# apache/arrow-go

Hardware: AMD Instinct MI355X
Metric: GB/s processed per kernel (Sum/Add/Filter/Take) vs HBM roofline (higher is better)
Workload: dtype int64+f64

## Files before the change

arrow_go_amd/csrc/ah_common.h:

```cpp
#pragma once
#include <hip/hip_runtime.h>
#include <initializer_list>
#include <type_traits>
#include <stdarg.h>
#include <stdint.h>
#include <stddef.h>
#include <stdio.h>
#include <stdlib.h>
#include <string.h>
#include "../../include/arrowhip.h"

#define AH_EXPORT extern "C" __attribute__((visibility("default")))

struct ah_filter_cache {
  bool valid;
  const uint8_t *fdata, *fvalid;
  int64_t foff, n, ntiles;
  int null_sel, tile_rows;
  void* buf;
  size_t bytes;
  int64_t* super_off;
  int* tile_local;
  int64_t* total;
};

struct ah_ctx {
  int device;
  hipStream_t stream;
  hipStream_t copy_stream;
  bool owns_stream;
  hipEvent_t ev_copy;
  hipEvent_t ev_compute;
  hipEvent_t t0, t1;
  hipEvent_t* marks;
  int n_marks;
  void* scratch;
  size_t scratch_bytes;
  void* temp;
  size_t temp_bytes;
  void* pack;
  size_t pack_bytes;
  uint64_t* pinned;
  uint64_t* dscalars;
  int num_cu;
  int tune_nt;
  int tune_blocks_per_cu;
  int opt_take_binned, opt_take_window_log2, opt_take_gather_wg, opt_take_gather_load, opt_take_gather_lds;
  int opt_groupby_keys;
  int opt_groupby_partition;
  int opt_encode_partition;
  int opt_encode_part_slots;
  int opt_encode_byte_map;
  int opt_encode_early_look;
  int opt_encode_part_min;
  int opt_hash_direct;
  int opt_hash_sum_partition;
  int opt_sort_msd;
  int opt_scan_segment_log2;
  void* expr_cache;
  int capturing;
  ah_filter_cache fcache;
  int opt_scan_onepass;
  void* scan_recs;
  size_t scan_recs_bytes;
  unsigned scan_epoch;
  int opt_groupby_seed;
  int opt_groupby_reserve;
  int opt_groupby_lean;
  int opt_filter_cache;
  int take_clustered_hint;
  int opt_take_vec;
  bool take_hint_valid, take_hint_live;
  const void* take_hint_idx; int64_t take_hint_nidx; int take_hint_kind, take_hint_near, take_hint_uses, opt_take_hint_cache;
  unsigned long long take_hint_word;
  int opt_arith_xcd_map;
  int opt_groupby_scale_guess;
  int opt_encode_unperm2_group;
  int opt_encode_resolve_wgs;
  int opt_encode_dict_compact;
  int opt_encode_table_batch;
  int opt_encode_unperm_group;
  int opt_take_vec_nt;
  unsigned long long* mailbox;
  unsigned long long mailbox_seq;
  char err[512];
};

static inline unsigned ah_stream_grid(const ah_ctx* c, int64_t work_items, int default_bpc = 8) {
  int bpc = c->tune_blocks_per_cu > 0 ? c->tune_blocks_per_cu : default_bpc;
  int64_t cap = bpc > 0 ? (int64_t)c->num_cu * bpc : ((int64_t)1 << 30);
  int64_t g = work_items < cap ? work_items : cap;
  return (unsigned)(g < 1 ? 1 : g);
}

static inline int ah_fail(ah_ctx* ctx, int code, const char* fmt, ...) __attribute__((format(printf, 3, 4)));
static inline int ah_fail(ah_ctx* ctx, int code, const char* fmt, ...) {
  if (ctx) {
    va_list ap;
    va_start(ap, fmt);
    vsnprintf(ctx->err, sizeof(ctx->err), fmt, ap);
    va_end(ap);
  }
  return code;
}

#define AH_HIP(ctx, call)                                                              \
  do {                                                                                 \
    hipError_t e__ = (call);                                                           \
    if (e__ != hipSuccess)                                                             \
      return ah_fail((ctx), AH_EHIP, "%s failed: %s (%s:%d)", #call, hipGetErrorString(e__), \
                     __FILE__, __LINE__);                                              \
  } while (0)

#define AH_ENTER_KEEP(ctx)                                             \
  do {                                                                 \
    if (!(ctx)) return AH_EINVALID;                                    \
    (ctx)->err[0] = 0;                                                 \
    AH_HIP((ctx), hipSetDevice((ctx)->device));                        \
  } while (0)

#define AH_ENTER(ctx)                                                  \
  do {                                                                 \
    AH_ENTER_KEEP(ctx);                                                \
    (ctx)->fcache.valid = false;                                       \
    (ctx)->take_hint_valid = false;                                    \
  } while (0)

static inline bool ah_take_hint_overlaps(const ah_ctx* c, const void* p, size_t nbytes) {
  if (!c->take_hint_valid || !c->take_hint_idx) return false;
  const uintptr_t a = (uintptr_t)p, b = a + nbytes, lo = (uintptr_t)c->take_hint_idx, hi = lo + (size_t)c->take_hint_nidx * (size_t)(c->take_hint_kind / 2);
  return a < hi && lo < b;
}
static inline bool ah_fcache_overlaps(const ah_ctx* c, const void* p, size_t nbytes) {
  if (!c->fcache.valid) return false;
  const uintptr_t a = (uintptr_t)p, b = a + nbytes;
  const uintptr_t lo = (uintptr_t)(c->fcache.foff >> 3), hi = (uintptr_t)((c->fcache.foff + c->fcache.n + 7) >> 3);
  for (const uint8_t* bm : {c->fcache.fdata, c->fcache.fvalid})
    if (bm && a < (uintptr_t)bm + hi && (uintptr_t)bm + lo < b) return true;
  return false;
}

#define AH_LAUNCH_CHECK(ctx) AH_HIP((ctx), hipGetLastError())

void ah_expr_cache_free(ah_ctx* ctx);
int ah_arith_binary(ah_ctx* ctx, int type, int op, int shape, const void* l, const void* r, void* out, int64_t len);
int ah_partition_by_group(ah_ctx* ctx, const int32_t* ids, const unsigned long long* vals, const uint8_t* vvalid, int64_t voff, int64_t n,
                          int shift, int passes, unsigned* hist, unsigned* offs, unsigned long long* alt_vals, unsigned* alt_ids,
                          unsigned long long* out_vals, unsigned* out_ids);
int ah_sort_rest_msd(ah_ctx* ctx, unsigned long long* keys, unsigned* rows, unsigned long long* alt_keys, unsigned* alt_rows, int64_t n,
                     unsigned long long varying, unsigned long long kmin, unsigned long long kmax, int float_bytes, int descending, void* tmp,
                     unsigned long long* out64, int* used);
size_t ah_sort_msd_temp_bytes(int64_t n);
int ah_sort_pairs_lsd(ah_ctx* ctx, unsigned long long* keys, unsigned* rows, unsigned long long* alt_keys, unsigned* alt_rows, int64_t n,
                      unsigned* hist, unsigned* offs, unsigned long long** sorted_keys);
int ah_take_binned_try(ah_ctx* ctx, int byte_width, const void* values, const uint8_t* vvalid, int64_t voff, int64_t nvalues, int iw,
                       int is_signed, const void* idx, const uint8_t* ivalid, int64_t ioff, int64_t nidx, void* out_values,
                       uint8_t* out_valid, unsigned long long* first_bad, int* used);
int ah_groupby_partitioned_try(ah_ctx* ctx, int is_f64, const uint64_t* keys, const uint8_t* kvalid, int64_t koff, const void* vals,
                               const uint8_t* vvalid, int64_t voff, int64_t n, uint64_t* out_keys, void* out_sums, int64_t* out_counts,
                               int64_t* out_first_rows, int64_t* out_ngroups, int32_t* out_null_group, int* used);
int ah_fused_f64_parts_dev(ah_ctx* ctx, int cmpop, const double* x, const uint8_t* valid, int64_t off, int64_t n, double threshold,
                           double* out_sum_dev, int64_t* out_count_dev, double* out_parts_dev);
size_t ah_sum_partial_bytes(int is_f64);
int ah_sum_chunk_partials(ah_ctx* ctx, int is_f64, const void* buf, size_t len, void* partials, int max_partials, int* n_written);
int ah_sum_finish_partials(ah_ctx* ctx, int is_f64, const void* partials, int n, void* res_dev);
int ah_sum_short_f64(ah_ctx* ctx, const void* buf, size_t len, void* res_dev);
int ah_encode_partitioned_try(ah_ctx* ctx, const uint64_t* keys, const uint8_t* valid, int64_t off, int64_t n, int encode_nulls, int lp, int slots,
                              int32_t* out_ids, uint64_t* out_dict, int64_t* out_first_rows, int64_t* out_ndict, int32_t* out_null_id, int* used);
int ah_encode_u64_groups(ah_ctx* ctx, const uint64_t* keys, const uint8_t* kvalid, int64_t koff, int64_t n, int32_t* ids, uint64_t* out_keys,
                         int64_t* out_first_rows, int64_t* out_ngroups, int32_t* out_null_group);
int ah_encode_u64_first_seen(ah_ctx* ctx, const uint64_t* keys, const uint8_t* valid, int64_t off, int64_t n, int32_t* ids, int64_t* out_first_rows,
                             int64_t* out_ngroups);
int ah_encode_tuple_first_seen(ah_ctx* ctx, int ncols, const ah_group_key* keys, int64_t n, int32_t* ids, int64_t* out_first_rows, int64_t* out_ngroups);
int ah_encode_first_look(ah_ctx* ctx, const uint64_t* keys, const uint8_t* valid, int64_t off, int64_t rows, uint64_t* distinct);
int ah_encode_partitioned2_try(ah_ctx* ctx, const uint64_t* keys, const uint8_t* valid, int64_t off, int64_t n, int encode_nulls, int lp, int slots,
                               int32_t* out_ids, uint64_t* out_dict, int64_t* out_first_rows, int64_t* out_ndict, int32_t* out_null_id, int* used);
int ah_compact_u64_by_bits(ah_ctx* ctx, const uint64_t* values, const uint8_t* bits, int64_t n, uint64_t* out_values, int64_t* out_rows);
int ah_check_stall(ah_ctx* ctx);
int ah_mailbox_read(ah_ctx* ctx, const unsigned long long* dev_words, int nwords, unsigned long long* out_host);
int ah_mailbox_begin(ah_ctx* ctx, unsigned long long** mb_out, unsigned long long* seq_out);
int ah_mailbox_wait(ah_ctx* ctx, unsigned long long seq, int nwords, unsigned long long* out_host);
#if defined(__HIPCC__)
__device__ __forceinline__ void ah_mailbox_post(unsigned long long* mb, unsigned long long seq, const unsigned long long* words, int nwords) {
  for (int i = 0; i < nwords; i++) __hip_atomic_store(&mb[i], words[i], __ATOMIC_RELAXED, __HIP_MEMORY_SCOPE_SYSTEM);
  __hip_atomic_store(&mb[7], seq, __ATOMIC_RELEASE, __HIP_MEMORY_SCOPE_SYSTEM);
}
#endif
int ah_mailbox_read2(ah_ctx* ctx, const unsigned long long* dev_words, int nwords, const unsigned long long* dev_words2, int nwords2,
                     unsigned long long* out_host);
int ah_scratch_reserve(ah_ctx* ctx, size_t nbytes, void** out);
int ah_temp_reserve(ah_ctx* ctx, size_t nbytes, void** out, bool* out_of_memory = nullptr);
int ah_pack_reserve(ah_ctx* ctx, size_t nbytes, void** out);
static inline constexpr size_t ah_pad(size_t b) { return (b + 255) & ~(size_t)255; }
struct TempCarver {
  uint8_t* base = nullptr;
  size_t used = 0;
  uint8_t* take(size_t b) { uint8_t* q = base ? base + used : nullptr; used += ah_pad(b); return q; }
  template <typename T> size_t take(T*& p, size_t count) { p = (T*)take(count * sizeof(T)); return ah_pad(count * sizeof(T)); }
};
constexpr int kDsScalars = 64;
constexpr int kDsSum = 0;
constexpr int kDsFusedSum = 8, kDsFusedCount = 9;
constexpr int kDsMinMax = 12;
constexpr int kDsGbDone = 20;
constexpr int kDsGbFlags = 21, kDsGbTotal = 22, kDsGbNullId = 23;
constexpr int kDsGbRange = 28;
constexpr int kDsEncFlags = 30, kDsEncTotal = 31, kDsEncNullId = 32;
constexpr int kDsEncLook = 33, kDsEncLookDone = 34;
constexpr int kDsEncLargest = 35, kDsEncLargestDone = 36;
constexpr int kDsPopcountPartials = kDsScalars;
constexpr int kPopcountMaxPartials = 4096;
int ah_popcount_async(ah_ctx* ctx, const uint8_t* bits, int64_t off, int64_t nbits, unsigned long long* total_dev);
int ah_popcount_post(ah_ctx* ctx, const uint8_t* bits, int64_t off, int64_t nbits, unsigned long long* total_dev, const unsigned long long* extra_dev,
                     unsigned long long* out_host );
int ah_zero_bytes(ah_ctx* ctx, void* dptr, size_t nbytes);

static inline int ah_type_width(int type) {
  switch (type) {
    case AH_UINT8: case AH_INT8: return 1;
    case AH_UINT16: case AH_INT16: return 2;
    case AH_UINT32: case AH_INT32: case AH_FLOAT32: return 4;
    case AH_UINT64: case AH_INT64: case AH_FLOAT64: return 8;
  }
  return 0;
}

static inline int64_t ah_ceil_div(int64_t a, int64_t b) { return (a + b - 1) / b; }

template <typename T> struct TypeTag { using type = T; };
template <class F>
inline bool with_numeric_type(int type, F&& f) {
  switch (type) {
    case AH_UINT8: f(TypeTag<uint8_t>{}); return true;
    case AH_INT8: f(TypeTag<int8_t>{}); return true;
    case AH_UINT16: f(TypeTag<uint16_t>{}); return true;
    case AH_INT16: f(TypeTag<int16_t>{}); return true;
    case AH_UINT32: f(TypeTag<uint32_t>{}); return true;
    case AH_INT32: f(TypeTag<int32_t>{}); return true;
    case AH_UINT64: f(TypeTag<uint64_t>{}); return true;
    case AH_INT64: f(TypeTag<int64_t>{}); return true;
    case AH_FLOAT32: f(TypeTag<float>{}); return true;
    case AH_FLOAT64: f(TypeTag<double>{}); return true;
  }
  return false;
}
template <class F>
inline bool with_numeric_carrier(int type, F&& f) {
  return with_numeric_type(type, [&](auto t) {
    using T = typename decltype(t)::type;
    if constexpr (__is_floating_point(T)) f(t);
    else f(TypeTag<typename std::make_unsigned<T>::type>{});
  });
}

static inline int ah_flag_clear(ah_ctx* c, unsigned* flag) {
  AH_HIP(c, hipMemsetAsync(flag, 0, sizeof(unsigned), c->stream));
  return AH_OK;
}
static inline int ah_flag_read(ah_ctx* c, const unsigned* flag, unsigned* bits) {
  AH_HIP(c, hipMemcpyAsync(c->pinned, flag, sizeof(unsigned), hipMemcpyDeviceToHost, c->stream));
  AH_HIP(c, hipStreamSynchronize(c->stream));
  *bits = *(volatile unsigned*)c->pinned;
  return AH_OK;
}
int ah_error_of_flag(ah_ctx* ctx, unsigned bits);

#define AH_WAVE 64

template <typename T>
struct alignas(sizeof(T)) ah_vec16 {
  T v[16 / sizeof(T)];
};

template <typename T>
using ah_raw16 __attribute__((aligned(sizeof(T)))) = T __attribute__((ext_vector_type(16 / sizeof(T))));
template <typename T>
__device__ __forceinline__ ah_vec16<T> ah_ld16_nt(const T* p) {
  const ah_raw16<T> raw = __builtin_nontemporal_load(reinterpret_cast<const ah_raw16<T>*>(p));
  ah_vec16<T> r;
#pragma unroll
  for (int j = 0; j < (int)(16 / sizeof(T)); j++) r.v[j] = raw[j];
  return r;
}
template <typename T>
__device__ __forceinline__ void ah_st16_nt(T* p, const ah_vec16<T>& x) {
  ah_raw16<T> raw;
#pragma unroll
  for (int j = 0; j < (int)(16 / sizeof(T)); j++) raw[j] = x.v[j];
  __builtin_nontemporal_store(raw, reinterpret_cast<ah_raw16<T>*>(p));
}

template <typename T>
__device__ __forceinline__ ah_vec16<T> ah_ld16(const T* p) {
  const ah_raw16<T> raw = *reinterpret_cast<const ah_raw16<T>*>(p);
  ah_vec16<T> r;
#pragma unroll
  for (int j = 0; j < (int)(16 / sizeof(T)); j++) r.v[j] = raw[j];
  return r;
}
template <typename T>
__device__ __forceinline__ void ah_st16(T* p, const ah_vec16<T>& x) {
  ah_raw16<T> raw;
#pragma unroll
  for (int j = 0; j < (int)(16 / sizeof(T)); j++) raw[j] = x.v[j];
  *reinterpret_cast<ah_raw16<T>*>(p) = raw;
}

template <typename T>
using ah_aligned16 = T __attribute__((ext_vector_type(16 / sizeof(T))));
template <typename ST>
__device__ __forceinline__ ah_vec16<ST> ah_load16(const ST* base, int64_t i, bool aligned) {
  ah_vec16<ST> v;
  if (aligned) {
    const ah_aligned16<ST> t = __builtin_nontemporal_load((const ah_aligned16<ST>*)base + i);
    __builtin_memcpy(&v, &t, 16);
  } else {
    v = ah_ld16<ST>(base + i * (int64_t)(16 / sizeof(ST)));
  }
  return v;
}
template <typename ST>
__device__ __forceinline__ void ah_store16(ST* base, int64_t i, const ah_vec16<ST>& v, bool aligned) {
  if (aligned) {
    ah_aligned16<ST> t;
    __builtin_memcpy(&t, &v, 16);
    __builtin_nontemporal_store(t, (ah_aligned16<ST>*)base + i);
  } else {
    ah_st16<ST>(base + i * (int64_t)(16 / sizeof(ST)), v);
  }
}

template <typename T>
__device__ __forceinline__ T ah_wave_sum(T v) {
#pragma unroll
  for (int o = 32; o > 0; o >>= 1) v += __shfl_down(v, o, 64);
  return v;
}
template <typename T>
__device__ __forceinline__ T ah_wave_max(T v) {
#pragma unroll
  for (int o = 32; o > 0; o >>= 1) {
    const T t = __shfl_down(v, o, 64);
    v = t > v ? t : v;
  }
  return v;
}
template <typename A, typename B>
__device__ __forceinline__ void ah_wave_max2(A& a, B& b) {
#pragma unroll
  for (int o = 32; o > 0; o >>= 1) {
    const A ta = __shfl_down(a, o, 64);
    const B tb = __shfl_down(b, o, 64);
    a = ta > a ? ta : a;
    b = tb > b ? tb : b;
  }
}

__device__ __forceinline__ int ah_lane() { return (int)(threadIdx.x & 63); }

__device__ __forceinline__ int ah_bit(const uint8_t* __restrict__ bm, int64_t i) {
  return bm == nullptr ? 1 : (bm[i >> 3] >> (i & 7)) & 1;
}

__device__ __forceinline__ uint64_t ah_load_bits64(const uint8_t* __restrict__ bm, int64_t pos, int nvalid);
__device__ __forceinline__ uint64_t ah_wave_bits64(const uint8_t* __restrict__ bm, int64_t pos0, int64_t nrows_left) {
  const int64_t p = ((int64_t)__builtin_amdgcn_readfirstlane((int)(pos0 >> 32)) << 32) | (unsigned)__builtin_amdgcn_readfirstlane((int)pos0);
  const int64_t left = ((int64_t)__builtin_amdgcn_readfirstlane((int)(nrows_left >> 32)) << 32) | (unsigned)__builtin_amdgcn_readfirstlane((int)nrows_left);
  return ah_load_bits64(bm, p, left >= 64 ? 64 : (int)(left < 0 ? 0 : left));
}
__device__ __forceinline__ uint64_t ah_load_bits64(const uint8_t* __restrict__ bm, int64_t pos, int nvalid) {
  uint64_t mask = nvalid >= 64 ? ~0ull : ((1ull << nvalid) - 1);
  if (nvalid <= 0) return 0;
  if (bm == nullptr) return mask;
  uintptr_t addr = (uintptr_t)bm + (uintptr_t)(pos >> 3);
  uintptr_t base = addr & ~(uintptr_t)7;
  int shift = (int)((addr - base) * 8 + (pos & 7));
  const uint64_t* w = (const uint64_t*)base;
  uint64_t lo = w[0] >> shift;
  if (shift != 0 && shift + nvalid > 64) lo |= w[1] << (64 - shift);
  return lo & mask;
}

__device__ __forceinline__ void put_bits(uint8_t* __restrict__ bm, int64_t pos, unsigned long long word, int cnt) {
  const uintptr_t addr = (uintptr_t)bm + (uintptr_t)(pos >> 3);
  const int sub = (int)(pos & 7);
  if (cnt == 64 && sub == 0 && (addr & 7) == 0) {
    *(unsigned long long*)addr = word;
    return;
  }
  const uintptr_t base = addr & ~(uintptr_t)3;
  int shift = (int)((addr - base) * 8) + sub;
  const unsigned long long m = cnt >= 64 ? ~0ull : ((1ull << cnt) - 1);
  word &= m;
  unsigned* w = (unsigned*)base;
  const unsigned long long mlo = m << shift, vlo = word << shift;
  const unsigned long long mhi = shift ? (m >> (64 - shift)) : 0ull, vhi = shift ? (word >> (64 - shift)) : 0ull;
  const unsigned m0 = (unsigned)mlo, m1 = (unsigned)(mlo >> 32), m2 = (unsigned)mhi;
  const unsigned v0 = (unsigned)vlo, v1 = (unsigned)(vlo >> 32), v2 = (unsigned)vhi;
  if (m0) { atomicAnd(&w[0], ~m0); if (v0) atomicOr(&w[0], v0); }
  if (m1) { atomicAnd(&w[1], ~m1); if (v1) atomicOr(&w[1], v1); }
  if (m2) { atomicAnd(&w[2], ~m2); if (v2) atomicOr(&w[2], v2); }
}

__device__ __forceinline__ void put_word(uint8_t* __restrict__ out, int64_t out_off, int aligned, int64_t chunk, unsigned long long word, int cnt) {
  if (aligned && cnt == 64) *(unsigned long long*)(out + (out_off + chunk * 64) / 8) = word;
  else put_bits(out, out_off + chunk * 64, word, cnt);
}

__device__ __forceinline__ void put_chunk_bytes(uint8_t* __restrict__ bm, int64_t chunk, int64_t n, unsigned long long word) {
  const int64_t left = n - chunk * 64;
  const int nbytes = left >= 64 ? 8 : (int)((left + 7) >> 3);
  for (int b = 0; b < nbytes; b++) bm[chunk * 8 + b] = (uint8_t)(word >> (8 * b));
}
```

arrow_go_amd/csrc/ah_ctx.hip:

```cpp
#include <chrono>
#include "ah_common.h"

static const char* kVersion = "arrowhip 0.1 (gfx950)";

AH_EXPORT const char* ah_version(void) { return kVersion; }

AH_EXPORT int ah_device_count(int* n_host) {
  int n = 0;
  hipError_t e = hipGetDeviceCount(&n);
  if (n_host) *n_host = (e == hipSuccess) ? n : 0;
  return e == hipSuccess ? AH_OK : AH_EHIP;
}

static int ctx_init_common(ah_ctx* c) {
  AH_HIP(c, hipStreamCreateWithFlags(&c->copy_stream, hipStreamNonBlocking));
  AH_HIP(c, hipEventCreateWithFlags(&c->ev_copy, hipEventDisableTiming));
  AH_HIP(c, hipEventCreateWithFlags(&c->ev_compute, hipEventDisableTiming));
  AH_HIP(c, hipEventCreate(&c->t0));
  AH_HIP(c, hipEventCreate(&c->t1));
  AH_HIP(c, hipHostMalloc((void**)&c->pinned, 64 * sizeof(uint64_t), hipHostMallocDefault));
  AH_HIP(c, hipMalloc((void**)&c->dscalars, (kDsScalars + kPopcountMaxPartials) * sizeof(uint64_t)));
  AH_HIP(c, hipMemset(c->dscalars, 0, (kDsScalars + kPopcountMaxPartials) * sizeof(uint64_t)));
  AH_HIP(c, hipHostMalloc((void**)&c->mailbox, 256, hipHostMallocCoherent | hipHostMallocMapped));
  memset(c->mailbox, 0, 256);
  hipDeviceProp_t prop;
  AH_HIP(c, hipGetDeviceProperties(&prop, c->device));
  c->num_cu = prop.multiProcessorCount > 0 ? prop.multiProcessorCount : 256;
  const char* e_nt = getenv("ARROWHIP_NT");
  c->tune_nt = e_nt ? atoi(e_nt) : 1;
  const char* e_bpc = getenv("ARROWHIP_BLOCKS_PER_CU");
  c->tune_blocks_per_cu = e_bpc ? atoi(e_bpc) : 0;
  auto env_int = [](const char* name, int dflt) { const char* e = getenv(name); return e ? atoi(e) : dflt; };
  c->opt_take_binned = env_int("ARROWHIP_TAKE_BINNED", 1);
  c->opt_take_window_log2 = env_int("ARROWHIP_TAKE_WINDOW_LOG2", 22);
  c->opt_take_gather_wg = env_int("ARROWHIP_TAKE_GATHER_WG_PER_CU", 8);
  c->opt_groupby_partition = env_int("ARROWHIP_GROUPBY_PARTITION", 1);
  c->opt_groupby_keys = env_int("ARROWHIP_GROUPBY_KEYS", 1280);
  c->opt_hash_direct = env_int("ARROWHIP_HASH_DIRECT", 2);
  c->opt_hash_sum_partition = env_int("ARROWHIP_HASH_PARTITION", 1);
  c->opt_encode_partition = env_int("ARROWHIP_ENCODE_PARTITION", 1);
  c->opt_encode_part_min = env_int("ARROWHIP_ENCODE_PART_MIN", 300000);
  c->opt_encode_early_look = env_int("ARROWHIP_ENCODE_EARLY_LOOK", 1);
  c->opt_encode_byte_map = env_int("ARROWHIP_ENCODE_BYTE_MAP", 1);
  c->opt_encode_part_slots = env_int("ARROWHIP_ENCODE_PART_SLOTS", 8192);
  c->opt_sort_msd = env_int("ARROWHIP_SORT_MSD", 1);
  c->opt_scan_segment_log2 = env_int("ARROWHIP_SCAN_SEGMENT_LOG2", 0);
  c->opt_take_gather_lds = env_int("ARROWHIP_TAKE_GATHER_LDS", 1);
  c->opt_take_vec_nt = env_int("ARROWHIP_TAKE_VEC_NT", 7);
  c->opt_encode_unperm_group = env_int("ARROWHIP_ENCODE_UNPERM_GROUP", 4);
  c->opt_encode_table_batch = env_int("ARROWHIP_ENCODE_TABLE_BATCH", 1);
  c->opt_encode_dict_compact = env_int("ARROWHIP_ENCODE_DICT_COMPACT", 1);
  c->opt_encode_resolve_wgs = env_int("ARROWHIP_ENCODE_RESOLVE_WGS", 1024);
  c->opt_encode_unperm2_group = env_int("ARROWHIP_ENCODE_UNPERM2_GROUP", 4);
  c->opt_groupby_scale_guess = env_int("ARROWHIP_GROUPBY_SCALE_GUESS", 1);
  c->opt_arith_xcd_map = env_int("ARROWHIP_ARITH_XCD_MAP", 0);
  c->opt_take_vec = env_int("ARROWHIP_TAKE_VEC", 1);
  c->opt_take_gather_load = env_int("ARROWHIP_TAKE_GATHER_LOAD", 0);
  return AH_OK;
}

static int ctx_create(int device_id, void* stream, bool borrow, ah_ctx** out) {
  if (!out) return AH_EINVALID;
  *out = nullptr;
  ah_ctx* c = (ah_ctx*)calloc(1, sizeof(ah_ctx));
  if (!c) return AH_EINVALID;
  c->device = device_id;
  hipError_t e = hipSetDevice(device_id);
  if (e != hipSuccess) { free(c); return AH_EHIP; }
  if (borrow) {
    c->stream = (hipStream_t)stream;
    c->owns_stream = false;
  } else {
    e = hipStreamCreateWithFlags(&c->stream, hipStreamNonBlocking);
    if (e != hipSuccess) { free(c); return AH_EHIP; }
    c->owns_stream = true;
  }
  int rc = ctx_init_common(c);
  if (rc != AH_OK) { fprintf(stderr, "arrowhip: ctx init failed: %s\n", c->err); free(c); return rc; }
  c->opt_filter_cache = c->owns_stream ? 1 : 0;
  c->opt_take_hint_cache = c->owns_stream ? 1 : 0;
  c->opt_groupby_lean = 1;
  c->opt_scan_onepass = 1;
  c->opt_groupby_seed = 1;
  c->opt_groupby_reserve = 1;
  *out = c;
  return AH_OK;
}

AH_EXPORT int ah_ctx_create(int device_id, ah_ctx** out) { return ctx_create(device_id, nullptr, false, out); }
AH_EXPORT int ah_ctx_create_on_stream(int device_id, void* hip_stream, ah_ctx** out) {
  return ctx_create(device_id, hip_stream, true, out);
}

AH_EXPORT void ah_ctx_destroy(ah_ctx* c) {
  if (!c) return;
  (void)hipSetDevice(c->device);
  (void)hipStreamSynchronize(c->stream);
  (void)hipStreamSynchronize(c->copy_stream);
  ah_expr_cache_free(c);
  if (c->scratch) (void)hipFree(c->scratch);
  if (c->pinned) (void)hipHostFree(c->pinned);
  if (c->dscalars) (void)hipFree(c->dscalars);
  if (c->mailbox) (void)hipHostFree(c->mailbox);
  if (c->fcache.buf) (void)hipFree(c->fcache.buf);
  if (c->scan_recs) (void)hipFree(c->scan_recs);
  if (c->temp) (void)hipFree(c->temp);
  if (c->pack) (void)hipFree(c->pack);
  (void)hipEventDestroy(c->ev_copy);
  (void)hipEventDestroy(c->ev_compute);
  (void)hipEventDestroy(c->t0);
  (void)hipEventDestroy(c->t1);
  for (int i = 0; i < c->n_marks; i++) if (c->marks[i]) (void)hipEventDestroy(c->marks[i]);
  free(c->marks);
  (void)hipStreamDestroy(c->copy_stream);
  if (c->owns_stream) (void)hipStreamDestroy(c->stream);
  free(c);
}

AH_EXPORT int ah_ctx_set_option(ah_ctx* c, const char* name, int64_t value) {
  AH_ENTER(c);
  if (!name) return ah_fail(c, AH_EINVALID, "set_option: null name");
  if (!strcmp(name, "nt")) c->tune_nt = (int)value;
  else if (!strcmp(name, "blocks_per_cu")) c->tune_blocks_per_cu = (int)value;
  else if (!strcmp(name, "take_binned")) c->opt_take_binned = (int)value;
  else if (!strcmp(name, "take_window_log2")) c->opt_take_window_log2 = (int)value;
  else if (!strcmp(name, "take_gather_wg_per_cu")) c->opt_take_gather_wg = (int)value;
  else if (!strcmp(name, "take_gather_lds")) c->opt_take_gather_lds = (int)value;
  else if (!strcmp(name, "take_vec")) c->opt_take_vec = (int)value;
  else if (!strcmp(name, "take_hint_cache")) { c->opt_take_hint_cache = (int)value; c->take_hint_valid = false; }
  else if (!strcmp(name, "take_vec_nt")) c->opt_take_vec_nt = (int)value;
  else if (!strcmp(name, "encode_unperm_group")) c->opt_encode_unperm_group = (int)value;
  else if (!strcmp(name, "encode_table_batch")) c->opt_encode_table_batch = (int)value;
  else if (!strcmp(name, "encode_dict_compact")) c->opt_encode_dict_compact = (int)value;
  else if (!strcmp(name, "encode_unperm2_group")) c->opt_encode_unperm2_group = (int)value;
  else if (!strcmp(name, "encode_resolve_wgs")) c->opt_encode_resolve_wgs = value < 1 ? 1 : (int)value;
  else if (!strcmp(name, "groupby_scale_guess")) c->opt_groupby_scale_guess = (int)value;
  else if (!strcmp(name, "arith_xcd_map")) c->opt_arith_xcd_map = (int)value;
  else if (!strcmp(name, "take_gather_load")) c->opt_take_gather_load = (int)value;
  else if (!strcmp(name, "groupby_partition")) c->opt_groupby_partition = (int)value;
  else if (!strcmp(name, "groupby_keys")) c->opt_groupby_keys = (int)value;
  else if (!strcmp(name, "hash_direct")) c->opt_hash_direct = (int)value;
  else if (!strcmp(name, "hash_sum_partition")) c->opt_hash_sum_partition = (int)value;
  else if (!strcmp(name, "encode_partition")) c->opt_encode_partition = (int)value;
  else if (!strcmp(name, "encode_part_min")) c->opt_encode_part_min = (int)value;
  else if (!strcmp(name, "encode_early_look")) c->opt_encode_early_look = (int)value;
  else if (!strcmp(name, "encode_byte_map")) c->opt_encode_byte_map = (int)value;
  else if (!strcmp(name, "encode_part_slots")) c->opt_encode_part_slots = (int)value;
  else if (!strcmp(name, "sort_msd")) c->opt_sort_msd = (int)value;
  else if (!strcmp(name, "scan_onepass")) c->opt_scan_onepass = (int)value;
  else if (!strcmp(name, "groupby_lean")) c->opt_groupby_lean = (int)value;
  else if (!strcmp(name, "groupby_seed")) c->opt_groupby_seed = (int)value;
  else if (!strcmp(name, "groupby_reserve")) c->opt_groupby_reserve = (int)value;
  else if (!strcmp(name, "filter_cache")) { c->opt_filter_cache = value != 0; if (!value) c->fcache.valid = false; }
  else if (!strcmp(name, "scan_segment_log2")) c->opt_scan_segment_log2 = (int)value;
  else return ah_fail(c, AH_EINVALID, "set_option: unknown option '%s'", name);
  return AH_OK;
}

AH_EXPORT const char* ah_last_error(ah_ctx* c) { return c ? c->err : "null context"; }

namespace {
__global__ void mailbox_post_kernel(const unsigned long long* __restrict__ src, int nwords, const unsigned long long* __restrict__ src2, int nwords2,
                                    unsigned long long* mailbox, unsigned long long seq) {
  for (int i = 0; i < nwords; i++) __hip_atomic_store(&mailbox[i], src[i], __ATOMIC_RELAXED, __HIP_MEMORY_SCOPE_SYSTEM);
  for (int i = 0; i < nwords2; i++) __hip_atomic_store(&mailbox[nwords + i], src2[i], __ATOMIC_RELAXED, __HIP_MEMORY_SCOPE_SYSTEM);
  __hip_atomic_store(&mailbox[7], seq, __ATOMIC_RELEASE, __HIP_MEMORY_SCOPE_SYSTEM);
}
}
int ah_mailbox_read(ah_ctx* c, const unsigned long long* dev_words, int nwords, unsigned long long* out_host) {
  return ah_mailbox_read2(c, dev_words, nwords, nullptr, 0, out_host);
}
int ah_mailbox_begin(ah_ctx* c, unsigned long long** mb_out, unsigned long long* seq_out) {
  if (c->capturing) { c->capturing = 2; return ah_fail(c, AH_EINVALID, "this call returns a value to the host: it cannot be recorded into a graph"); }
  *mb_out = c->mailbox + 8;
  *seq_out = ++c->mailbox_seq;
  return AH_OK;
}
int ah_mailbox_wait(ah_ctx* c, unsigned long long seq, int nwords, unsigned long long* out_host) {
  if (nwords < 1 || nwords > 7) return ah_fail(c, AH_EINVALID, "mailbox_wait: 1..7 words");
  unsigned long long* mb = c->mailbox + 8;
  bool seen = false;
  const auto t0 = std::chrono::steady_clock::now();
  for (unsigned spin = 0;; spin++) {
    if (__atomic_load_n(&mb[7], __ATOMIC_ACQUIRE) == seq) { seen = true; break; }
    __builtin_ia32_pause();
    if ((spin & 1023u) == 1023u && std::chrono::steady_clock::now() - t0 > std::chrono::milliseconds(5)) break;
  }
  if (!seen) {
    AH_HIP(c, hipStreamSynchronize(c->stream));
    if (__atomic_load_n(&mb[7], __ATOMIC_ACQUIRE) != seq) return ah_fail(c, AH_EHIP, "mailbox_wait: the kernel did not report");
  }
  for (int i = 0; i < nwords; i++) out_host[i] = __atomic_load_n(&mb[i], __ATOMIC_RELAXED);
  return AH_OK;
}
int ah_mailbox_read2(ah_ctx* c, const unsigned long long* dev_words, int nwords, const unsigned long long* dev_words2, int nwords2,
                     unsigned long long* out_host) {
  if (nwords < 1 || nwords2 < 0 || nwords + nwords2 > 7) return ah_fail(c, AH_EINVALID, "mailbox_read: 1..7 words");
  if (c->capturing) { c->capturing = 2; return ah_fail(c, AH_EINVALID, "this call returns a value to the host: it cannot be recorded into a graph"); }
  unsigned long long* mb = c->mailbox + 8;
  const unsigned long long seq = ++c->mailbox_seq;
  mailbox_post_kernel<<<1, 1, 0, c->stream>>>(dev_words, nwords, dev_words2, nwords2, mb, seq);
  AH_LAUNCH_CHECK(c);
  bool seen = false;
  const auto t0 = std::chrono::steady_clock::now();
  for (unsigned spin = 0;; spin++) {
    if (__atomic_load_n(&mb[7], __ATOMIC_ACQUIRE) == seq) { seen = true; break; }
    __builtin_ia32_pause();
    if ((spin & 1023u) == 1023u && std::chrono::steady_clock::now() - t0 > std::chrono::milliseconds(5)) break;
  }
  if (!seen) {
    AH_HIP(c, hipStreamSynchronize(c->stream));
    if (__atomic_load_n(&mb[7], __ATOMIC_ACQUIRE) != seq) return ah_fail(c, AH_EHIP, "mailbox_read: the post kernel did not report");
  }
  for (int i = 0; i < nwords + nwords2; i++) out_host[i] = __atomic_load_n(&mb[i], __ATOMIC_RELAXED);
  return AH_OK;
}

int ah_scratch_reserve(ah_ctx* c, size_t nbytes, void** out) {
  if (nbytes > c->scratch_bytes) {
    AH_HIP(c, hipStreamSynchronize(c->stream));
    if (c->scratch) AH_HIP(c, hipFree(c->scratch));
    c->scratch = nullptr;
    c->scratch_bytes = 0;
    size_t want = (nbytes + ((size_t)1 << 20) - 1) & ~(((size_t)1 << 20) - 1);
    AH_HIP(c, hipMalloc(&c->scratch, want));
    c->scratch_bytes = want;
  }
  *out = c->scratch;
  return AH_OK;
}

int ah_temp_reserve(ah_ctx* c, size_t nbytes, void** out, bool* out_of_memory) {
  if (out_of_memory) *out_of_memory = false;
  if (nbytes > c->temp_bytes) {
    AH_HIP(c, hipStreamSynchronize(c->stream));
    if (c->temp) AH_HIP(c, hipFree(c->temp));
    c->temp = nullptr;
    c->temp_bytes = 0;
    size_t want = (nbytes + ((size_t)1 << 20) - 1) & ~(((size_t)1 << 20) - 1);
    if (hipMalloc(&c->temp, want) != hipSuccess) { (void)hipGetLastError(); if (out_of_memory) *out_of_memory = true; return ah_fail(c, AH_EHIP, "out of device memory (%zu bytes of temporaries)", want); }
    c->temp_bytes = want;
  }
  *out = c->temp;
  return AH_OK;
}

int ah_pack_reserve(ah_ctx* c, size_t nbytes, void** out) {
  if (nbytes > c->pack_bytes) {
    AH_HIP(c, hipStreamSynchronize(c->stream));
    if (c->pack) AH_HIP(c, hipFree(c->pack));
    c->pack = nullptr;
    c->pack_bytes = 0;
    size_t want = (nbytes + ((size_t)1 << 20) - 1) & ~(((size_t)1 << 20) - 1);
    if (hipMalloc(&c->pack, want) != hipSuccess) { (void)hipGetLastError(); return ah_fail(c, AH_EHIP, "out of device memory (%zu bytes of packed keys)", want); }
    c->pack_bytes = want;
  }
  *out = c->pack;
  return AH_OK;
}

AH_EXPORT int ah_buf_alloc(ah_ctx* c, size_t nbytes, void** dptr_host) {
  AH_ENTER_KEEP(c);
  if (!dptr_host) return ah_fail(c, AH_EINVALID, "ah_buf_alloc: null out pointer");
  *dptr_host = nullptr;
  if (nbytes == 0) nbytes = 1;
  nbytes = (nbytes + 63) & ~(size_t)63;
  AH_HIP(c, hipMalloc(dptr_host, nbytes));
  return AH_OK;
}

AH_EXPORT int ah_buf_free(ah_ctx* c, void* dptr) {
  AH_ENTER(c);
  if (dptr) AH_HIP(c, hipFree(dptr));
  return AH_OK;
}

AH_EXPORT int ah_host_alloc_pinned(ah_ctx* c, size_t nbytes, void** hptr_host) {
  AH_ENTER_KEEP(c);
  if (!hptr_host) return ah_fail(c, AH_EINVALID, "ah_host_alloc_pinned: null out pointer");
  if (nbytes == 0) nbytes = 1;
  nbytes = (nbytes + 63) & ~(size_t)63;
  AH_HIP(c, hipHostMalloc(hptr_host, nbytes, hipHostMallocDefault));
  return AH_OK;
}

AH_EXPORT int ah_host_free_pinned(ah_ctx* c, void* hptr) {
  AH_ENTER_KEEP(c);
  if (hptr) AH_HIP(c, hipHostFree(hptr));
  return AH_OK;
}

AH_EXPORT int ah_upload_async(ah_ctx* c, void* dptr, const void* hptr, size_t nbytes) {
  AH_ENTER_KEEP(c);
  if (ah_fcache_overlaps(c, dptr, nbytes)) c->fcache.valid = false;
  if (ah_take_hint_overlaps(c, dptr, nbytes)) c->take_hint_valid = false;
  if (nbytes == 0) return AH_OK;
  AH_HIP(c, hipEventRecord(c->ev_compute, c->stream));
  AH_HIP(c, hipStreamWaitEvent(c->copy_stream, c->ev_compute, 0));
  AH_HIP(c, hipMemcpyAsync(dptr, hptr, nbytes, hipMemcpyHostToDevice, c->copy_stream));
  AH_HIP(c, hipEventRecord(c->ev_copy, c->copy_stream));
  AH_HIP(c, hipStreamWaitEvent(c->stream, c->ev_copy, 0));
  return AH_OK;
}

AH_EXPORT int ah_download_async(ah_ctx* c, void* hptr, const void* dptr, size_t nbytes) {
  AH_ENTER_KEEP(c);
  if (nbytes == 0) return AH_OK;
  AH_HIP(c, hipEventRecord(c->ev_compute, c->stream));
  AH_HIP(c, hipStreamWaitEvent(c->copy_stream, c->ev_compute, 0));
  AH_HIP(c, hipMemcpyAsync(hptr, dptr, nbytes, hipMemcpyDeviceToHost, c->copy_stream));
  AH_HIP(c, hipEventRecord(c->ev_copy, c->copy_stream));
  AH_HIP(c, hipStreamWaitEvent(c->stream, c->ev_copy, 0));
  return AH_OK;
}

AH_EXPORT int ah_memset_async(ah_ctx* c, void* dptr, int byte_value, size_t nbytes) {
  AH_ENTER_KEEP(c);
  if (ah_fcache_overlaps(c, dptr, nbytes)) c->fcache.valid = false;
  if (ah_take_hint_overlaps(c, dptr, nbytes)) c->take_hint_valid = false;
  if (nbytes == 0) return AH_OK;
  AH_HIP(c, hipMemsetAsync(dptr, byte_value, nbytes, c->stream));
  return AH_OK;
}

namespace {
typedef unsigned zero_v4 __attribute__((ext_vector_type(4)));
__global__ __launch_bounds__(256) void zero_bytes_kernel(uint8_t* __restrict__ p, size_t n) {
  const size_t head = ((16 - ((uintptr_t)p & 15)) & 15) < n ? ((16 - ((uintptr_t)p & 15)) & 15) : n;
  const size_t body = (n - head) / 16, tail0 = head + body * 16;
  const size_t i = (size_t)blockIdx.x * 256 + threadIdx.x;
  if (i < head) p[i] = 0;
  if (i < n - tail0) p[tail0 + i] = 0;
  zero_v4* q = (zero_v4*)(p + head);
  const zero_v4 z = {0u, 0u, 0u, 0u};
  for (size_t j = i; j < body; j += (size_t)gridDim.x * 256) q[j] = z;
}
}

int ah_zero_bytes(ah_ctx* c, void* dptr, size_t nbytes) {
  if (nbytes == 0) return AH_OK;
  const size_t want = (nbytes / 16 + 255) / 256 + 1;
  zero_bytes_kernel<<<(unsigned)(want < 4096 ? want : 4096), 256, 0, c->stream>>>((uint8_t*)dptr, nbytes);
  AH_LAUNCH_CHECK(c);
  return AH_OK;
}

namespace {
constexpr int kCopyBlock = 256, kCopyUnroll = 4;
typedef unsigned copy_v4 __attribute__((ext_vector_type(4)));
__global__ __launch_bounds__(kCopyBlock) void copy16_kernel(const copy_v4* __restrict__ src, copy_v4* __restrict__ dst, int64_t nvec) {
  const int64_t i = (int64_t)blockIdx.x * kCopyBlock * kCopyUnroll + threadIdx.x;
  if (i + (int64_t)(kCopyUnroll - 1) * kCopyBlock < nvec) {
    copy_v4 x[kCopyUnroll];
#pragma unroll
    for (int k = 0; k < kCopyUnroll; k++) x[k] = __builtin_nontemporal_load(&src[i + (int64_t)k * kCopyBlock]);
#pragma unroll
    for (int k = 0; k < kCopyUnroll; k++) __builtin_nontemporal_store(x[k], &dst[i + (int64_t)k * kCopyBlock]);
  } else {
#pragma unroll
    for (int k = 0; k < kCopyUnroll; k++) {
      const int64_t j = i + (int64_t)k * kCopyBlock;
      if (j < nvec) dst[j] = src[j];
    }
  }
}
}

AH_EXPORT int ah_copy_async(ah_ctx* c, void* dst, const void* src, size_t nbytes) {
  AH_ENTER_KEEP(c);
  if (ah_fcache_overlaps(c, dst, nbytes)) c->fcache.valid = false;
  if (ah_take_hint_overlaps(c, dst, nbytes)) c->take_hint_valid = false;
  if (nbytes == 0) return AH_OK;
  if (!dst || !src) return ah_fail(c, AH_EINVALID, "copy: null buffer");
  const uintptr_t d = (uintptr_t)dst, s = (uintptr_t)src;
  const bool disjoint = d + nbytes <= s || s + nbytes <= d;
  if (nbytes >= ((size_t)1 << 20) && ((d | s) & 15) == 0 && disjoint) {
    const int64_t nvec = (int64_t)(nbytes / 16);
    copy16_kernel<<<(unsigned)ah_ceil_div(nvec, (int64_t)kCopyBlock * kCopyUnroll), kCopyBlock, 0, c->stream>>>((const copy_v4*)src, (copy_v4*)dst, nvec);
    AH_LAUNCH_CHECK(c);
    const size_t done = (size_t)nvec * 16;
    if (done < nbytes) AH_HIP(c, hipMemcpyAsync((uint8_t*)dst + done, (const uint8_t*)src + done, nbytes - done, hipMemcpyDeviceToDevice, c->stream));
    return AH_OK;
  }
  AH_HIP(c, hipMemcpyAsync(dst, src, nbytes, hipMemcpyDeviceToDevice, c->stream));
  return AH_OK;
}

int ah_check_stall(ah_ctx* c) {
  if (!c->mailbox || !__atomic_load_n(&c->mailbox[16], __ATOMIC_ACQUIRE)) return AH_OK;
  __atomic_store_n(&c->mailbox[16], 0ull, __ATOMIC_RELAXED);
  return ah_fail(c, AH_EHIP, "cumulative_sum: a tile's look-back gave up waiting for a predecessor (results of that call are invalid)");
}

AH_EXPORT int ah_sync(ah_ctx* c) {
  AH_ENTER_KEEP(c);
  AH_HIP(c, hipStreamSynchronize(c->copy_stream));
  AH_HIP(c, hipStreamSynchronize(c->stream));
  return ah_check_stall(c);
}

AH_EXPORT int ah_timer_start(ah_ctx* c) {
  AH_ENTER_KEEP(c);
  AH_HIP(c, hipEventRecord(c->t0, c->stream));
  return AH_OK;
}

AH_EXPORT int ah_timer_stop(ah_ctx* c, float* ms_host) {
  AH_ENTER_KEEP(c);
  AH_HIP(c, hipEventRecord(c->t1, c->stream));
  AH_HIP(c, hipEventSynchronize(c->t1));
  float ms = 0.f;
  AH_HIP(c, hipEventElapsedTime(&ms, c->t0, c->t1));
  if (ms_host) *ms_host = ms;
  return AH_OK;
}

AH_EXPORT int ah_event_record(ah_ctx* c, int slot) {
  AH_ENTER_KEEP(c);
  if (slot < 0 || slot >= (1 << 16)) return ah_fail(c, AH_EINVALID, "event_record: slot out of range");
  if (slot >= c->n_marks) {
    int n = c->n_marks ? c->n_marks : 64;
    while (n <= slot) n *= 2;
    hipEvent_t* m = (hipEvent_t*)realloc(c->marks, (size_t)n * sizeof(hipEvent_t));
    if (!m) return ah_fail(c, AH_EINVALID, "event_record: out of memory");
    for (int i = c->n_marks; i < n; i++) m[i] = nullptr;
    c->marks = m;
    c->n_marks = n;
  }
  if (!c->marks[slot]) AH_HIP(c, hipEventCreate(&c->marks[slot]));
  AH_HIP(c, hipEventRecord(c->marks[slot], c->stream));
  return AH_OK;
}

AH_EXPORT int ah_event_elapsed_ms(ah_ctx* c, int slot_a, int slot_b, float* ms_host) {
  AH_ENTER_KEEP(c);
  if (slot_a < 0 || slot_b < 0 || slot_a >= c->n_marks || slot_b >= c->n_marks || !c->marks[slot_a] || !c->marks[slot_b])
    return ah_fail(c, AH_EINVALID, "event_elapsed_ms: slot never recorded");
  AH_HIP(c, hipEventSynchronize(c->marks[slot_b]));
  float ms = 0.f;
  AH_HIP(c, hipEventElapsedTime(&ms, c->marks[slot_a], c->marks[slot_b]));
  if (ms_host) *ms_host = ms;
  return AH_OK;
}

AH_EXPORT int ah_wait_event(ah_ctx* c, void* hip_event_ptr) {
  AH_ENTER_KEEP(c);
  if (!hip_event_ptr) return AH_OK;
  AH_HIP(c, hipStreamWaitEvent(c->stream, *(hipEvent_t*)hip_event_ptr, 0));
  return AH_OK;
}

AH_EXPORT int ah_device_id(ah_ctx* c) { return c ? c->device : -1; }


struct ah_graph {
  ah_ctx* ctx;
  hipGraph_t graph;
  hipGraphExec_t exec;
  void* scratch;
  void* temp;
};

AH_EXPORT int ah_graph_begin(ah_ctx* c) {
  AH_ENTER(c);
  if (c->capturing) return ah_fail(c, AH_EINVALID, "graph_begin: already capturing");
  AH_HIP(c, hipStreamBeginCapture(c->stream, hipStreamCaptureModeRelaxed));
  c->capturing = 1;
  return AH_OK;
}

AH_EXPORT int ah_graph_end(ah_ctx* c, ah_graph** out) {
  if (!c) return AH_EINVALID;
  c->err[0] = 0;
  if (!out) return ah_fail(c, AH_EINVALID, "graph_end: null out pointer");
  *out = nullptr;
  if (!c->capturing) return ah_fail(c, AH_EINVALID, "graph_end: not capturing");
  const bool poisoned = c->capturing == 2;
  c->capturing = 0;
  hipGraph_t g = nullptr;
  hipError_t e = hipStreamEndCapture(c->stream, &g);
  if (e == hipSuccess && g && poisoned) {
    (void)hipGraphDestroy(g);
    return ah_fail(c, AH_EINVALID, "graph_end: a recorded call needed a value on the host — nothing was run, the capture is dropped");
  }
  if (e != hipSuccess || !g) {
    (void)hipGetLastError();
    return ah_fail(c, AH_EHIP, "graph_end: the capture was invalidated (%s) — a captured call waited for the device or allocated", hipGetErrorString(e));
  }
  hipGraphExec_t x = nullptr;
  e = hipGraphInstantiate(&x, g, nullptr, nullptr, 0);
  if (e != hipSuccess) { (void)hipGraphDestroy(g); return ah_fail(c, AH_EHIP, "graph_end: hipGraphInstantiate failed: %s", hipGetErrorString(e)); }
  ah_graph* r = (ah_graph*)calloc(1, sizeof(ah_graph));
  if (!r) { (void)hipGraphExecDestroy(x); (void)hipGraphDestroy(g); return ah_fail(c, AH_EINVALID, "graph_end: out of memory"); }
  r->ctx = c; r->graph = g; r->exec = x;
  r->scratch = c->scratch; r->temp = c->temp;
  *out = r;
  return AH_OK;
}

AH_EXPORT int ah_graph_launch(ah_ctx* c, ah_graph* g) {
  AH_ENTER(c);
  if (!g || g->ctx != c) return ah_fail(c, AH_EINVALID, "graph_launch: not a graph of this context");
  if (c->capturing) return ah_fail(c, AH_EINVALID, "graph_launch: the context is capturing");
  if (g->scratch != c->scratch || g->temp != c->temp)
    return ah_fail(c, AH_EINVALID, "graph_launch: a call since the recording grew one of the context's work areas (the recorded launches point into the old block) — record the sequence again");
  AH_HIP(c, hipGraphLaunch(g->exec, c->stream));
  return AH_OK;
}

AH_EXPORT int ah_graph_destroy(ah_graph* g) {
  if (!g) return AH_OK;
  (void)hipSetDevice(g->ctx->device);
  (void)hipStreamSynchronize(g->ctx->stream);
  (void)hipGraphExecDestroy(g->exec);
  (void)hipGraphDestroy(g->graph);
  free(g);
  return AH_OK;
}
```

arrow_go_amd/csrc/ah_msd.h:

```cpp
#pragma once
#include "ah_common.h"
#include "ah_bins.h"

namespace {

constexpr int kMsTile = 4096;
constexpr int kMsRows = kMsTile / kThreads;
constexpr int kMaxNb2 = 2048;

struct TileRange { int64_t lo, hi, id; int parent; };
__device__ __forceinline__ int ms_parent_of(int j, int nparents) { const int per = nparents >> 3; return ((j % per) << 3) | (j / per); }
__device__ __forceinline__ unsigned ms_tiles_of(const unsigned* __restrict__ pstart, const unsigned* __restrict__ pend, int j, int nparents) {
  const int p = ms_parent_of(j, nparents);
  return ((pend ? pend[p] : pstart[p + 1]) - pstart[p] + kMsTile - 1) / kMsTile;
}
__device__ __forceinline__ void ms_parent_tiles(const unsigned* __restrict__ pstart, const unsigned* __restrict__ pend, int nparents, unsigned* s_cnt,
                                                unsigned* s_start, unsigned* s_wsum) {
  const int t = threadIdx.x;
  s_cnt[t] = t < nparents ? ms_tiles_of(pstart, pend, t, nparents) : 0u;
  __syncthreads();
  block_excl_scan(s_cnt, s_start, s_wsum, nparents);
}
__device__ __forceinline__ long long ms_block_tile(unsigned b, unsigned nblocks, int nparents, const unsigned* s_cnt, const unsigned* s_start) {
  const int per = nparents >> 3;
  const unsigned x = b & 7, q = b >> 3, nblk = nblocks >> 3;
  auto class_lo = [&](unsigned c) { return s_start[c * per]; };
  auto class_n = [&](unsigned c) { return (c == 7 ? s_start[nparents - 1] + s_cnt[nparents - 1] : s_start[(c + 1) * per]) - s_start[c * per]; };
  long long g = -1;
  if (q < class_n(x)) {
    g = class_lo(x) + q;
  } else {
    unsigned spare = q - class_n(x);
    for (unsigned c = 0; c < x; c++) spare += nblk > class_n(c) ? nblk - class_n(c) : 0u;
    for (unsigned c = 0; c < 8 && g < 0; c++) {
      const unsigned surplus = class_n(c) > nblk ? class_n(c) - nblk : 0u;
      if (spare < surplus) g = class_lo(c) + nblk + spare; else spare -= surplus;
    }
  }
  return g;
}
__device__ __forceinline__ TileRange ms_tile_of_parent(const unsigned* __restrict__ pstart, const unsigned* __restrict__ pend, int nparents, int j, long long g,
                                                       const unsigned* s_start) {
  TileRange r;
  const int p = ms_parent_of(j, nparents);
  const int64_t b0 = pstart[p], b1 = pend ? pend[p] : pstart[p + 1];
  r.lo = b0 + (int64_t)(g - s_start[j]) * kMsTile;
  r.hi = r.lo + kMsTile < b1 ? r.lo + kMsTile : b1;
  r.id = g;
  r.parent = p;
  return r;
}
__device__ __forceinline__ TileRange ms_tile(const unsigned* __restrict__ pstart, int nparents, int64_t n, unsigned* s_cnt, unsigned* s_start,
                                             unsigned* s_wsum, int* s_pick, const unsigned* __restrict__ pend = nullptr) {
  TileRange r{0, 0, 0, -1};
  if (!pstart) {
    const int64_t tile = xcd_contiguous_tile((n + kMsTile - 1) / kMsTile);
    if (tile >= 0) { r.lo = tile * kMsTile; r.hi = r.lo + kMsTile < n ? r.lo + kMsTile : n; r.id = tile; r.parent = 0; }
    return r;
  }
  const int t = threadIdx.x;
  if (t == 0) *s_pick = -1;
  ms_parent_tiles(pstart, pend, nparents, s_cnt, s_start, s_wsum);
  const long long g = ms_block_tile(blockIdx.x, gridDim.x, nparents, s_cnt, s_start);
  if (g >= 0 && t < nparents && s_cnt[t] && s_start[t] <= g && g < s_start[t] + s_cnt[t]) *s_pick = t;
  __syncthreads();
  const int j = *s_pick;
  return j < 0 ? r : ms_tile_of_parent(pstart, pend, nparents, j, g, s_start);
}

__global__ __launch_bounds__(kThreads) void ms_tile_table_kernel(const unsigned* __restrict__ pstart, const unsigned* __restrict__ pend, int nparents,
                                                                  unsigned nblocks, TileRange* __restrict__ table) {
  __shared__ unsigned s_cnt[kThreads], s_start[kThreads], s_wsum[kThreads / 64];
  ms_parent_tiles(pstart, pend, nparents, s_cnt, s_start, s_wsum);
  const unsigned b = blockIdx.x * (unsigned)kThreads + threadIdx.x;
  if (b >= nblocks) return;
  const long long g = ms_block_tile(b, nblocks, nparents, s_cnt, s_start);
  TileRange r{0, 0, 0, -1};
  if (g >= 0) {
    int lo = 0, hi = nparents - 1;
    while (lo < hi) { const int mid = (lo + hi + 1) >> 1; if ((long long)s_start[mid] <= g) lo = mid; else hi = mid - 1; }
    int j = lo;
    while (j > 0 && !s_cnt[j]) j--;
    if (s_cnt[j] && (long long)s_start[j] <= g && g < (long long)s_start[j] + s_cnt[j]) r = ms_tile_of_parent(pstart, pend, nparents, j, g, s_start);
  }
  table[b] = r;
}

template <typename DIGIT>
__global__ __launch_bounds__(kThreads) void tile_hist_kernel(DIGIT dg, int64_t n, const unsigned* __restrict__ pstart, int nparents, int nb,
                                                              unsigned* __restrict__ cnt, const TileRange* __restrict__ tile_table = nullptr) {
  __shared__ unsigned s_h[DIGIT::kMaxDigits];
  __shared__ unsigned s_cnt[kThreads], s_start[kThreads], s_wsum[kThreads / 64];
  __shared__ int s_pick;
  const TileRange r = tile_table ? tile_table[blockIdx.x] : ms_tile(pstart, nparents, n, s_cnt, s_start, s_wsum, &s_pick);
  if (r.parent < 0) return;
  for (int b = threadIdx.x; b < nb; b += kThreads) s_h[b] = 0;
  __syncthreads();
  unsigned d[kMsRows];
#pragma unroll
  for (int u = 0; u < kMsRows; u++) { const int64_t i = r.lo + u * kThreads + threadIdx.x; d[u] = i < r.hi ? dg.digit(i, r.parent) : 0u; }
#pragma unroll
  for (int u = 0; u < kMsRows; u++) { const int64_t i = r.lo + u * kThreads + threadIdx.x; if (i < r.hi) atomicAdd(&s_h[d[u]], 1u); }
  __syncthreads();
  for (int b = threadIdx.x; b < nb; b += kThreads) cnt[r.id * nb + b] = s_h[b];
}

__global__ __launch_bounds__(kThreads) void ms_offs2_kernel(const unsigned* __restrict__ cnt, const unsigned* __restrict__ pstart, int nparents, int nb,
                                                             unsigned* __restrict__ toffs, unsigned* __restrict__ bstart, int64_t n,
                                                             unsigned* __restrict__ largest = nullptr, unsigned* __restrict__ done = nullptr,
                                                             unsigned long long* mb = nullptr, unsigned long long seq = 0) {
  __shared__ unsigned s_cnt[kThreads], s_start[kThreads], s_wsum[kThreads / 64];
  __shared__ unsigned s_carry;
  const int t = threadIdx.x, p = blockIdx.x;
  ms_parent_tiles(pstart, nullptr, nparents, s_cnt, s_start, s_wsum);
  const int j = (p & 7) * (nparents >> 3) + (p >> 3);
  const int64_t vt0 = s_start[j], vt1 = vt0 + s_cnt[j];
  __syncthreads();
  const unsigned base = pstart[p];
  auto post_largest = [&](unsigned mine) {
    if (!largest) return;
    if (t == 0) s_carry = 0;
    __syncthreads();
    if (mine) atomicMax(&s_carry, mine);
    __syncthreads();
    if (t == 0) {
      atomicMax(largest, s_carry);
      __threadfence();
      if (atomicAdd(done, 1u) == gridDim.x - 1u) {
        __threadfence();
        const unsigned long long w = __hip_atomic_exchange(largest, 0u, __ATOMIC_RELAXED, __HIP_MEMORY_SCOPE_AGENT);
        __hip_atomic_store(done, 0u, __ATOMIC_RELAXED, __HIP_MEMORY_SCOPE_AGENT);
        ah_mailbox_post(mb, seq, &w, 1);
      }
    }
  };
  if (nb <= kThreads / 2) {
    const int d = t & (nb - 1), g = t / nb, G = kThreads / nb;
    const int64_t per = (vt1 - vt0 + G - 1) / G, a0 = vt0 + g * per, a1 = a0 + per < vt1 ? a0 + per : vt1;
    unsigned part = 0;
    for (int64_t vt = a0; vt < a1; vt++) part += cnt[vt * nb + d];
    s_cnt[t] = part;
    __syncthreads();
    unsigned before = 0, tot = 0;
    for (int gg = 0; gg < G; gg++) { const unsigned c = s_cnt[gg * nb + d]; before += gg < g ? c : 0u; tot += c; }
    __syncthreads();
    s_cnt[t] = t < nb ? tot : 0u;
    __syncthreads();
    block_excl_scan(s_cnt, s_start, s_wsum, nb);
    post_largest(t < nb ? tot : 0u);
    unsigned run = base + s_start[d] + before;
    if (g == 0) bstart[(int64_t)p * nb + d] = run;
    for (int64_t vt = a0; vt < a1; vt++) { toffs[vt * nb + d] = run; run += cnt[vt * nb + d]; }
    if (p == nparents - 1 && t == 0) bstart[(int64_t)nparents * nb] = (unsigned)n;
    return;
  }
  unsigned tot[2] = {0, 0};
  for (int64_t vt = vt0; vt < vt1; vt++)
    for (int h = 0; h < 2; h++) { const int d = t + h * kThreads; if (d < nb) tot[h] += cnt[vt * nb + d]; }
  unsigned excl[2];
  unsigned carry = 0;
  for (int h = 0; h < 2; h++) {
    if (h * kThreads >= nb) break;
    s_cnt[t] = t + h * kThreads < nb ? tot[h] : 0u;
    __syncthreads();
    block_excl_scan(s_cnt, s_start, s_wsum, kThreads);
    excl[h] = carry + s_start[t];
    if (t == kThreads - 1) s_carry = s_start[t] + s_cnt[t];
    __syncthreads();
    carry += s_carry;
    __syncthreads();
  }
  post_largest(tot[0] > tot[1] ? tot[0] : tot[1]);
  for (int h = 0; h < 2; h++) {
    const int d = t + h * kThreads;
    if (d >= nb) break;
    unsigned run = base + excl[h];
    bstart[(int64_t)p * nb + d] = run;
    for (int64_t vt = vt0; vt < vt1; vt++) { toffs[vt * nb + d] = run; run += cnt[vt * nb + d]; }
  }
  if (p == nparents - 1 && t == 0) bstart[(int64_t)nparents * nb] = (unsigned)n;
}

template <int CTRL>
__device__ __forceinline__ unsigned ms_dpp(unsigned v) { return (unsigned)__builtin_amdgcn_update_dpp((int)v, (int)v, CTRL, 0xF, 0xF, false); }
__device__ __forceinline__ unsigned ms_xor_lane(unsigned v, int j, int lane) {
  switch (j) {
    case 1: return ms_dpp<0xB1>(v);
    case 2: return ms_dpp<0x4E>(v);
    case 4: { const unsigned a = ms_dpp<0x124>(v), b = ms_dpp<0x12C>(v); return (lane & 4) ? a : b; }
    case 8: return ms_dpp<0x128>(v);
    case 16: { auto r = __builtin_amdgcn_permlane16_swap(v, v, false, false); return (lane & 16) ? r[0] : r[1]; }
    default: { auto r = __builtin_amdgcn_permlane32_swap(v, v, false, false); return (lane & 32) ? r[0] : r[1]; }
  }
}
template <typename E>
__device__ __forceinline__ E ms_pick(const E& mine, const E& other, bool keep_min) {
  const bool other_less = E::less(other, mine);
  return (other_less == keep_min) ? other : mine;
}

template <typename E, int SLOTS>
__device__ __forceinline__ void ms_bitonic(E (&x)[SLOTS], int lane) {
#pragma unroll
  for (int k = 2; k <= 64 * SLOTS; k <<= 1) {
#pragma unroll
    for (int j = k >> 1; j > 0; j >>= 1) {
      if (j >= 64) {
#pragma unroll
        for (int sl = 0; sl < SLOTS; sl++) {
          const int ps = sl ^ (j >> 6);
          if (ps > sl) {
            const bool asc = (sl & (k >> 6)) == 0;
            const bool swap = E::less(x[ps], x[sl]) == asc;
            const E a = x[sl], bb = x[ps];
            x[sl] = swap ? bb : a;
            x[ps] = swap ? a : bb;
          }
        }
      } else {
        const bool low = (lane & j) == 0;
#pragma unroll
        for (int sl = 0; sl < SLOTS; sl++) {
          const bool asc = k < 64 ? (lane & k) == 0 : (sl & (k >> 6)) == 0;
          x[sl] = ms_pick(x[sl], E::xchg(x[sl], j, lane), low == asc);
        }
      }
    }
  }
}
}
```

arrow_go_amd/csrc/ah_sort.hip:

```cpp
#include <algorithm>
#include <type_traits>
#include <vector>
#include "ah_sort_radix.h"

namespace {

enum { kCatRest = 0, kCatNaN = 1, kCatNull = 2 };

template <typename T>
__device__ __forceinline__ unsigned long long make_key(T v, bool descending) {
  using U = typename std::make_unsigned<typename std::conditional<std::is_floating_point<T>::value,
                                                                    typename std::conditional<sizeof(T) == 4, int, long long>::type, T>::type>::type;
  constexpr U sign = (U)1 << (sizeof(T) * 8 - 1);
  U k;
  if constexpr (std::is_floating_point<T>::value) {
    if (v == (T)0) v = (T)0;
    U b = __builtin_bit_cast(U, v);
    k = (b & sign) ? (U)~b : (U)(b | sign);
  } else if constexpr (std::is_signed<T>::value) {
    k = (U)v ^ sign;
  } else {
    k = (U)v;
  }
  if (descending) k = (U)~k;
  return (unsigned long long)k;
}

template <typename T>
struct Column {
  const T* values;
  const uint8_t* valid;
  int64_t off;
  int descending, nulls_at_start;
  const unsigned* rows_in;
  __device__ __forceinline__ void load(int64_t i, unsigned long long* key, unsigned* row, unsigned* digit) const {
    const unsigned r = rows_in ? rows_in[i] : (unsigned)i;
    const T v = values[r];
    int cat = kCatRest;
    if (!ah_bit(valid, off + r)) cat = kCatNull;
    else if (std::is_floating_point<T>::value && v != v) cat = kCatNaN;
    *key = cat == kCatRest ? make_key<T>(v, descending) : 0ull;
    *row = r;
    *digit = nulls_at_start ? (unsigned)(2 - cat) : (unsigned)cat;
  }
};
struct IdVal {
  const int32_t* ids;
  const unsigned long long* vals;
  const uint8_t* vvalid;
  int64_t voff;
  int shift;
  __device__ __forceinline__ void load(int64_t i, unsigned long long* key, unsigned* row, unsigned* digit) const {
    const unsigned g = (unsigned)ids[i];
    const bool ok = ah_bit(vvalid, voff + i);
    *key = ok ? vals[i] : 0ull;
    *row = ok ? g : (g | 0x80000000u);
    *digit = (g >> shift) & 255u;
  }
};

struct ValId {
  const unsigned long long* vals;
  const unsigned* ids;
  int shift;
  __device__ __forceinline__ void load(int64_t i, unsigned long long* key, unsigned* row, unsigned* digit) const {
    *key = vals[i];
    *row = ids[i];
    *digit = ((*row & 0x7fffffffu) >> shift) & 255u;
  }
};

template <typename T>
__global__ __launch_bounds__(kBlock) void pairs_kernel(const T* __restrict__ values, int64_t n, int descending, unsigned long long* __restrict__ keys,
                                                        unsigned* __restrict__ rows, unsigned long long* __restrict__ res) {
  KeyStats st;
  st.init();
  constexpr int U = 4;
  const int64_t stride = (int64_t)gridDim.x * kBlock * U;
  for (int64_t base = (int64_t)blockIdx.x * kBlock * U + threadIdx.x; base < n; base += stride) {
    T v[U];
#pragma unroll
    for (int u = 0; u < U; u++) { const int64_t i = base + (int64_t)u * kBlock; v[u] = i < n ? __builtin_nontemporal_load(&values[i]) : (T)0; }
#pragma unroll
    for (int u = 0; u < U; u++) {
      const int64_t i = base + (int64_t)u * kBlock;
      if (i >= n) continue;
      if (std::is_floating_point<T>::value && v[u] != v[u]) { st.nans++; continue; }
      const unsigned long long k = make_key<T>(v[u], descending);
      __builtin_nontemporal_store(k, &keys[i]);
      __builtin_nontemporal_store((unsigned)i, &rows[i]);
      st.add(k);
    }
  }
  st = ah_block_reduce<kBlock>(st);
  if (threadIdx.x == 0) st.store<5>(res + (size_t)blockIdx.x * 5);
}

__global__ __launch_bounds__(kBlock) void emit_kernel(const unsigned* __restrict__ rows, int64_t n, uint64_t* __restrict__ out) {
  const int64_t stride = (int64_t)gridDim.x * kBlock;
  for (int64_t i = (int64_t)blockIdx.x * kBlock + threadIdx.x; i < n; i += stride) out[i] = rows[i];
}


template <typename T>
int sort_by_column(ah_ctx* c, SortBuffers& b, const void* values, const uint8_t* valid, int64_t off, int64_t n, int descending,
                   int nulls_at_start, const unsigned* rows_in) {
  const int64_t ntiles = ah_ceil_div(n, (int64_t)kTile * tiles_per_block(n));
  int rc;
  Column<T> col{(const T*)values, valid, off, descending, nulls_at_start, rows_in};
  int64_t rest_lo = 0, rest_n = 0;
  unsigned long long k_and = ~0ull, k_or = 0, kmin = ~0ull, kmax = 0;
  bool have_stats = false;
  if (valid == nullptr && rows_in == nullptr && n >= ((int64_t)1 << 20)) {
    const unsigned pgrid = std::min(ah_stream_grid(c, ah_ceil_div(n, (int64_t)kBlock * 4), 8), (unsigned)kAndOrGrid);
    pairs_kernel<T><<<pgrid, kBlock, 0, c->stream>>>((const T*)values, n, descending, b.ka, b.ra, b.andor);
    AH_LAUNCH_CHECK(c);
    std::vector<unsigned long long> parts((size_t)pgrid * 5);
    AH_HIP(c, hipMemcpyAsync(parts.data(), b.andor, parts.size() * 8, hipMemcpyDeviceToHost, c->stream));
    AH_HIP(c, hipStreamSynchronize(c->stream));
    unsigned long long nans = 0;
    for (unsigned g = 0; g < pgrid; g++) {
      k_and &= parts[g * 5]; k_or |= parts[g * 5 + 1];
      kmin = parts[g * 5 + 2] < kmin ? parts[g * 5 + 2] : kmin;
      kmax = parts[g * 5 + 3] > kmax ? parts[g * 5 + 3] : kmax;
      nans += parts[g * 5 + 4];
    }
    if (nans == 0) { have_stats = true; rest_lo = 0; rest_n = n; }
  }
  if (!have_stats) {
    if ((rc = radix_pass(c, col, n, b.hist, b.offs, b.ka, b.ra)) != AH_OK) return rc;
    unsigned ends[3];
    for (int d = 0; d < 3; d++)
      AH_HIP(c, hipMemcpyAsync(&c->pinned[d], b.offs + ((int64_t)d + 1) * ntiles - 1, 4, hipMemcpyDeviceToHost, c->stream));
    AH_HIP(c, hipStreamSynchronize(c->stream));
    for (int d = 0; d < 3; d++) ends[d] = *(volatile unsigned*)&c->pinned[d];
    rest_lo = nulls_at_start ? ends[1] : 0;
    rest_n = nulls_at_start ? (int64_t)ends[2] - ends[1] : ends[0];
  }
  unsigned long long *kcur = b.ka + rest_lo, *kalt = b.kb + rest_lo;
  unsigned *rcur = b.ra + rest_lo, *ralt = b.rb + rest_lo;
  if (rest_n > 1) {
    if (!have_stats) {
      const unsigned agrid = std::min(ah_stream_grid(c, ah_ceil_div(rest_n, kBlock), 4), (unsigned)kAndOrGrid);
      and_or_kernel<<<agrid, kBlock, 0, c->stream>>>(kcur, rest_n, b.andor);
      AH_LAUNCH_CHECK(c);
      std::vector<unsigned long long> parts((size_t)agrid * 4);
      AH_HIP(c, hipMemcpyAsync(parts.data(), b.andor, parts.size() * 8, hipMemcpyDeviceToHost, c->stream));
      AH_HIP(c, hipStreamSynchronize(c->stream));
      for (unsigned g = 0; g < agrid; g++) {
        k_and &= parts[g * 4]; k_or |= parts[g * 4 + 1];
        kmin = parts[g * 4 + 2] < kmin ? parts[g * 4 + 2] : kmin;
        kmax = parts[g * 4 + 3] > kmax ? parts[g * 4 + 3] : kmax;
      }
    }
    const unsigned long long varying = k_and ^ k_or;
    int nvar = 0;
    for (int by = 0; by < (int)sizeof(T); by++) nvar += ((varying >> (8 * by)) & 0xFFull) != 0;
    bool done = false;
    if (rows_in == nullptr && nvar >= 4 && c->opt_sort_msd) {
      int used = -1;
      if ((rc = ah_sort_rest_msd(c, kcur, rcur, kalt, ralt, rest_n, varying, kmin, kmax, std::is_floating_point<T>::value ? (int)sizeof(T) : 0, descending, b.msd_tmp,
                                 (unsigned long long*)(rest_n == n ? b.final_out : nullptr), &used)) != AH_OK) return rc;
      if (used > 0) {
        done = true;
        b.emitted = rest_n == n && b.final_out != nullptr;
      } else if (used == 0 && b.msd_tmp && ah_sort_msd_temp_bytes(rest_n) != 0) {
        if ((rc = radix_pass(c, col, n, b.hist, b.offs, b.ka, b.ra)) != AH_OK) return rc;
      }
    }
    for (int by = 0; !done && by < (int)sizeof(T); by++) {
      if (((varying >> (8 * by)) & 0xFFull) == 0) continue;
      Pairs src{kcur, rcur, 8 * by};
      if ((rc = radix_pass(c, src, rest_n, b.hist, b.offs, kalt, ralt)) != AH_OK) return rc;
      unsigned long long* tk = kcur; kcur = kalt; kalt = tk;
      unsigned* tr = rcur; rcur = ralt; ralt = tr;
    }
    if (!b.emitted && rcur != b.ra + rest_lo) AH_HIP(c, hipMemcpyAsync(b.ra + rest_lo, rcur, (size_t)rest_n * 4, hipMemcpyDeviceToDevice, c->stream));
  }
  return AH_OK;
}

int sort_dispatch(ah_ctx* c, SortBuffers& b, const SortCol& k, int64_t n, const unsigned* rows_in) {
  switch (k.type) {
#define AH_SORT(ID, T) case ID: return sort_by_column<T>(c, b, k.values, k.valid, k.off, n, k.descending, k.nulls_at_start, rows_in);
    AH_SORT(AH_UINT8, uint8_t) AH_SORT(AH_INT8, int8_t) AH_SORT(AH_UINT16, uint16_t) AH_SORT(AH_INT16, int16_t)
    AH_SORT(AH_UINT32, uint32_t) AH_SORT(AH_INT32, int32_t) AH_SORT(AH_UINT64, uint64_t) AH_SORT(AH_INT64, int64_t)
    AH_SORT(AH_FLOAT32, float) AH_SORT(AH_FLOAT64, double)
#undef AH_SORT
  }
  if (ah_sort_is_binary(k.type)) return ah_sort_by_binary(c, b, k, n, rows_in);
  return ah_fail(c, AH_ENOTIMPL, "sorting not supported for type %d", k.type);
}

int sort_keys(ah_ctx* c, int nkeys, const SortCol* keys, int64_t n, uint64_t* out) {
  SortBuffers b;
  const int64_t ntiles = ah_ceil_div(n, kTile);
  int rc;
  bool any_binary = false;
  for (int k = 0; k < nkeys; k++) any_binary |= ah_sort_is_binary(keys[k].type);
  const size_t hist_bytes = (size_t)kRadix * ntiles * 4;
  const size_t msd_bytes = c->opt_sort_msd ? ah_sort_msd_temp_bytes(n) : 0;
  const size_t bin_bytes = any_binary ? kBinArrays * Carver::pad((size_t)n * 4) : 0;
  const size_t total = 2 * Carver::pad((size_t)n * 8) + (nkeys > 1 ? 3 : 2) * Carver::pad((size_t)n * 4) + 2 * Carver::pad(hist_bytes) + Carver::pad(4096 * 8 * 8) + Carver::pad(msd_bytes) + bin_bytes;
  void* arena;
  if ((rc = ah_temp_reserve(c, total, &arena)) != AH_OK) return rc;
  Carver tmp{(uint8_t*)arena};
  tmp.take((size_t)n * 8, &b.ka);
  tmp.take((size_t)n * 8, &b.kb);
  tmp.take((size_t)n * 4, &b.ra);
  tmp.take((size_t)n * 4, &b.rb);
  b.rc = nullptr;
  if (nkeys > 1) tmp.take((size_t)n * 4, &b.rc);
  tmp.take(hist_bytes, &b.hist);
  tmp.take(hist_bytes, &b.offs);
  tmp.take((size_t)kAndOrGrid * 8 * 8, &b.andor);
  if (msd_bytes) { uint8_t* m; tmp.take(msd_bytes, &m); b.msd_tmp = m; }
  if (any_binary)
    for (int i = 0; i < kBinArrays; i++) tmp.take((size_t)n * 4, &b.bin[i]);
  const unsigned* rows_in = nullptr;
  if (nkeys == 1) b.final_out = out;
  for (int k = nkeys - 1; k >= 0; k--) {
    if ((rc = sort_dispatch(c, b, keys[k], n, rows_in)) != AH_OK) return rc;
    if (k > 0) {
      AH_HIP(c, hipMemcpyAsync(b.rc, b.ra, (size_t)n * 4, hipMemcpyDeviceToDevice, c->stream));
      rows_in = b.rc;
    }
  }
  if (!b.emitted) {
    emit_kernel<<<ah_stream_grid(c, ah_ceil_div(n, kBlock), 8), kBlock, 0, c->stream>>>(b.ra, n, out);
    AH_LAUNCH_CHECK(c);
  }
  return AH_OK;
}

}

int ah_partition_by_group(ah_ctx* c, const int32_t* ids, const unsigned long long* vals, const uint8_t* vvalid, int64_t voff, int64_t n, int shift,
                          int passes, unsigned* hist, unsigned* offs, unsigned long long* alt_vals, unsigned* alt_ids,
                          unsigned long long* out_vals, unsigned* out_ids) {
  IdVal src{ids, vals, vvalid, voff, shift};
  if (passes == 1) return radix_pass(c, src, n, hist, offs, out_vals, out_ids);
  int rc = radix_pass(c, src, n, hist, offs, alt_vals, alt_ids);
  if (rc != AH_OK) return rc;
  ValId src2{alt_vals, alt_ids, shift + 8};
  return radix_pass(c, src2, n, hist, offs, out_vals, out_ids);
}

int ah_sort_pairs_lsd(ah_ctx* c, unsigned long long* keys, unsigned* rows, unsigned long long* alt_keys, unsigned* alt_rows, int64_t n,
                      unsigned* hist, unsigned* offs, unsigned long long** sorted_keys) {
  for (int by = 0; by < 8; by++) {
    Pairs src{keys, rows, 8 * by};
    int rc = radix_pass(c, src, n, hist, offs, alt_keys, alt_rows);
    if (rc != AH_OK) return rc;
    unsigned long long* tk = keys; keys = alt_keys; alt_keys = tk;
    unsigned* tr = rows; rows = alt_rows; alt_rows = tr;
  }
  *sorted_keys = keys;
  return AH_OK;
}

static int check_column(ah_ctx* c, int type, const void* values) {
  const int w = ah_type_width(type);
  if (!w) return ah_fail(c, AH_ENOTIMPL, "sorting not supported for type %d", type);
  if (!values) return ah_fail(c, AH_EINVALID, "sort_indices: null buffer");
  if ((uintptr_t)values & (uintptr_t)(w - 1)) return ah_fail(c, AH_EINVALID, "sort_indices: buffer not element-aligned");
  return AH_OK;
}

static int check_key(ah_ctx* c, const ah_sort_key& k, SortCol* col) {
  *col = SortCol{k.type, nullptr, nullptr, nullptr, 0, k.valid, k.off, k.descending, k.nulls_at_start};
  switch (k.type) {
    case AH_BINARY: case AH_LARGE_BINARY: {
      const int ow = k.type == AH_BINARY ? 4 : 8;
      if (!k.offsets) return ah_fail(c, AH_EINVALID, "sort_indices: null buffer");
      if ((uintptr_t)k.offsets & (uintptr_t)(ow - 1)) return ah_fail(c, AH_EINVALID, "sort_indices: buffer not element-aligned");
      col->offsets = k.offsets;
      col->data = (const uint8_t*)k.values;
      return AH_OK;
    }
    case AH_FIXED_SIZE_BINARY: case AH_DECIMAL128: case AH_DECIMAL256: {
      const int w = k.type == AH_DECIMAL128 ? 16 : k.type == AH_DECIMAL256 ? 32 : k.byte_width;
      if (k.byte_width != w || w < 1) return ah_fail(c, AH_EINVALID, "sort_indices: byte width %d does not fit type %d", k.byte_width, k.type);
      if (!k.values) return ah_fail(c, AH_EINVALID, "sort_indices: null buffer");
      col->data = (const uint8_t*)k.values;
      col->width = w;
      return AH_OK;
    }
  }
  const int rc = check_column(c, k.type, k.values);
  if (rc != AH_OK) return rc;
  col->values = (const uint8_t*)k.values + k.off * ah_type_width(k.type);
  return AH_OK;
}

AH_EXPORT int ah_sort_indices(ah_ctx* c, int type, const void* values, const uint8_t* valid, int64_t off, int64_t n, int descending,
                              int nulls_at_start, uint64_t* out_indices) {
  return ah_sort_indices_multi(c, 1, &type, &values, &valid, &off, n, &descending, &nulls_at_start, out_indices);
}

AH_EXPORT int ah_sort_indices_multi(ah_ctx* c, int nkeys, const int* types, const void* const* values, const uint8_t* const* valids,
                                    const int64_t* offs, int64_t n, const int* descending, const int* nulls_at_start, uint64_t* out_indices) {
  AH_ENTER(c);
  if (nkeys < 1) return ah_fail(c, AH_EINVALID, "must provide at least one sort key");
  if (n < 0) return ah_fail(c, AH_EINVALID, "sort_indices: negative length");
  for (int k = 0; k < nkeys; k++)
    if (offs[k] < 0) return ah_fail(c, AH_EINVALID, "sort_indices: negative offset");
  if (n == 0) return AH_OK;
  if (!out_indices) return ah_fail(c, AH_EINVALID, "sort_indices: null buffer");
  if (n >= ((int64_t)1 << 32)) return ah_fail(c, AH_ENOTIMPL, "sort_indices: more than 2^32 - 1 rows in one batch");
  std::vector<SortCol> cols((size_t)nkeys);
  for (int k = 0; k < nkeys; k++) {
    int rc = check_column(c, types[k], values[k]);
    if (rc != AH_OK) return rc;
    cols[k] = SortCol{types[k], values[k], nullptr, nullptr, 0, valids[k], offs[k], descending[k], nulls_at_start[k]};
  }
  return sort_keys(c, nkeys, cols.data(), n, out_indices);
}

AH_EXPORT int ah_sort_indices_keys(ah_ctx* c, int nkeys, const ah_sort_key* keys, int64_t n, uint64_t* out_indices) {
  AH_ENTER(c);
  if (nkeys < 1) return ah_fail(c, AH_EINVALID, "must provide at least one sort key");
  if (!keys) return ah_fail(c, AH_EINVALID, "sort_indices: null buffer");
  if (n < 0) return ah_fail(c, AH_EINVALID, "sort_indices: negative length");
  for (int k = 0; k < nkeys; k++)
    if (keys[k].off < 0) return ah_fail(c, AH_EINVALID, "sort_indices: negative offset");
  if (n == 0) return AH_OK;
  if (!out_indices) return ah_fail(c, AH_EINVALID, "sort_indices: null buffer");
  if (n >= ((int64_t)1 << 32)) return ah_fail(c, AH_ENOTIMPL, "sort_indices: more than 2^32 - 1 rows in one batch");
  std::vector<SortCol> cols((size_t)nkeys);
  for (int k = 0; k < nkeys; k++) {
    const int rc = check_key(c, keys[k], &cols[k]);
    if (rc != AH_OK) return rc;
  }
  return sort_keys(c, nkeys, cols.data(), n, out_indices);
}
```

arrow_go_amd/csrc/ah_sort_msd.hip:

```cpp
#include "ah_common.h"
#include "ah_bins.h"
#include "ah_msd.h"

namespace {

constexpr int kLocalMax = 512;
constexpr int kBigMax = 8192, kBigList = 1024;

struct MsMap {
  unsigned long long mask;
  int lshift;
  int fkind, descending;
};
__device__ __forceinline__ double ms_value(unsigned long long u, const MsMap& m) {
  if (m.fkind == 8) {
    const unsigned long long k = m.descending ? ~u : u;
    return __builtin_bit_cast(double, (k >> 63) ? (k & 0x7fffffffffffffffull) : ~k);
  }
  const unsigned k = m.descending ? ~(unsigned)(u >> 32) : (unsigned)(u >> 32);
  return (double)__builtin_bit_cast(float, (k >> 31) ? (k & 0x7fffffffu) : ~k);
}
__device__ __forceinline__ double ms_frac(unsigned long long u, unsigned long long pa, unsigned long long pb, const MsMap& m) {
  if (pb <= pa) return 0.0;
  if (m.fkind && m.lshift == (m.fkind == 8 ? 0 : 32) && ((pa ^ pb) >> 63)) {
    const double xa = ms_value(pa, m), xb = ms_value(pb, m);
    if (xb != xa && xa - xa == 0.0 && xb - xb == 0.0) return (ms_value(u, m) - xa) / (xb - xa);
  }
  return (double)(u - pa) / (double)(pb - pa);
}
constexpr int kSplit = 4096;
constexpr int64_t kSample = (int64_t)1 << 18;

__global__ __launch_bounds__(256) void ms_sample_kernel(const unsigned long long* __restrict__ keys, int64_t n, int64_t stride, int64_t count, MsMap m,
                                                         unsigned long long* __restrict__ sample, unsigned* __restrict__ sample_rows) {
  const int64_t j = (int64_t)blockIdx.x * 256 + threadIdx.x;
  if (j >= count) return;
  const int64_t i = j * stride;
  sample[j] = i < n ? (keys[i] & m.mask) << m.lshift : ~0ull;
  sample_rows[j] = (unsigned)j;
}
struct MsPoints {
  const unsigned long long* sorted;
  int64_t count;
  unsigned long long umin, umax;
  __device__ __forceinline__ unsigned long long at(int64_t i) const { return i <= 0 ? umin : (i > count ? umax : sorted[i - 1]); }
  __device__ __forceinline__ int64_t first(int k) const { return k == 0 ? 0 : 64 * (int64_t)k + 1; }
  __device__ __forceinline__ int64_t last(int k) const { return k == kSplit - 1 ? count + 1 : 64 * (int64_t)(k + 1) + 1; }
};
constexpr int kFlagWords = kSplit / 32;
__global__ __launch_bounds__(256) void ms_split_kernel(MsPoints p, unsigned long long* __restrict__ split, unsigned* __restrict__ flags) {
  const int k = blockIdx.x * 256 + threadIdx.x;
  if (k > kSplit) return;
  split[k] = k == kSplit ? p.umax : p.at(p.first(k));
  if (k == kSplit) return;
  const int64_t i0 = p.first(k), i1 = p.last(k);
  const unsigned long long a = p.at(i0), b = p.at(i1);
  bool flag = k == 0 || k == kSplit - 1;
  if (!flag && b > a) {
    const double w = (double)(b - a), g = (double)(i1 - i0);
    for (int64_t i = i0 + 1; i < i1; i++) {
      const double dev = (double)(p.at(i) - a) / w - (double)(i - i0) / g;
      flag = flag || dev > 0.25 || dev < -0.25;
    }
  }
  if (flag) atomicOr(&flags[k >> 5], 1u << (k & 31));
}

__global__ __launch_bounds__(256) void ms_dupes_kernel(const unsigned long long* __restrict__ sorted, int64_t count, int64_t run, unsigned* __restrict__ found) {
  const int64_t i = (int64_t)blockIdx.x * 256 + threadIdx.x;
  if (i + run < count && sorted[i] == sorted[i + run]) *found = 1u;
}

__global__ __launch_bounds__(256) void ms_guide_kernel(const unsigned long long* __restrict__ split, unsigned short* __restrict__ guide) {
  const int c = blockIdx.x * 256 + threadIdx.x;
  if (c > 4096) return;
  if (c == 4096) { guide[c] = (unsigned short)(kSplit - 1); return; }
  const unsigned long long v = (unsigned long long)c << 52;
  int lo = 0;
  for (int step = kSplit >> 1; step > 0; step >>= 1) lo += split[lo + step] <= v ? step : 0;
  guide[c] = (unsigned short)lo;
}

__global__ __launch_bounds__(kThreads) void ms_bucket_kernel(const unsigned long long* __restrict__ keys, int64_t n, MsMap m, MsPoints p,
                                                         const unsigned long long* __restrict__ split, const unsigned* __restrict__ flags,
                                                         const unsigned short* __restrict__ guide, unsigned per, unsigned* __restrict__ bucket) {
  __shared__ unsigned long long s_s[kSplit + 1];
  __shared__ unsigned s_f[kFlagWords];
  __shared__ unsigned short s_g[4097];
  for (int i = threadIdx.x; i <= kSplit; i += kThreads) { s_s[i] = split[i]; s_g[i] = guide[i]; }
  for (int i = threadIdx.x; i < kFlagWords; i += kThreads) s_f[i] = flags[i];
  __syncthreads();
  constexpr int U = 4;
  const int64_t stride = (int64_t)gridDim.x * kThreads * U;
  for (int64_t base = (int64_t)blockIdx.x * kThreads * U + threadIdx.x; base < n; base += stride) {
    unsigned long long u[U];
    unsigned lo[U], hi[U];
#pragma unroll
    for (int q = 0; q < U; q++) {
      const int64_t i = base + q * kThreads;
      u[q] = i < n ? (__builtin_nontemporal_load(&keys[i]) & m.mask) << m.lshift : s_s[0];
    }
#pragma unroll
    for (int q = 0; q < U; q++) { lo[q] = s_g[u[q] >> 52]; hi[q] = s_g[(u[q] >> 52) + 1]; }
    bool more = true;
    while (more) {
      more = false;
#pragma unroll
      for (int q = 0; q < U; q++) {
        if (lo[q] < hi[q]) {
          const unsigned mid = (lo[q] + hi[q] + 1) >> 1;
          if (s_s[mid] <= u[q]) lo[q] = mid; else hi[q] = mid - 1;
          more = more || lo[q] < hi[q];
        }
      }
    }
#pragma unroll
    for (int q = 0; q < U; q++) {
      const int64_t i = base + q * kThreads;
      if (i >= n) continue;
      double f;
      if ((s_f[lo[q] >> 5] >> (lo[q] & 31)) & 1u) {
        int64_t a = p.first((int)lo[q]), b = p.last((int)lo[q]);
        const double g = (double)(b - a);
        const int64_t a0 = a;
        unsigned long long pa = p.at(a), pb = p.at(b);
        while (b - a > 1) {
          const int64_t mid = (a + b) >> 1;
          const unsigned long long pm = p.at(mid);
          if (b - a <= 16) {
            const double d = ms_frac(pm, pa, pb, m) - (double)(mid - a) / (double)(b - a);
            if (d < 0.3 && d > -0.3) break;
          }
          if (pm <= u[q]) { a = mid; pa = pm; } else { b = mid; pb = pm; }
        }
        f = ((double)(a - a0) + ms_frac(u[q], pa, pb, m) * (double)(b - a)) / g;
      } else {
        const unsigned long long x = s_s[lo[q]], y = s_s[lo[q] + 1];
        f = y > x ? (double)(u[q] - x) * __builtin_amdgcn_rcp((double)(y - x)) : 0.0;
      }
      f = f >= 0.0 ? f : 0.0;
      unsigned in = (unsigned)(f * (double)per);
      in = in < per ? in : per - 1;
      __builtin_nontemporal_store(lo[q] * per + in, &bucket[i]);
    }
  }
}

struct MsDigit {
  static constexpr int kMaxDigits = kMaxNb2;
  const unsigned* bucket; int shift; unsigned mask;
  __device__ __forceinline__ unsigned digit(int64_t i, int) const { return (__builtin_nontemporal_load(&bucket[i]) >> shift) & mask; }
};

template <bool WITH_BUCKET>
__global__ __launch_bounds__(kThreads) void ms_scatter_kernel(const unsigned long long* __restrict__ keys, const unsigned* __restrict__ rows,
                                                               const unsigned* __restrict__ bucket, int64_t n, const unsigned* __restrict__ pstart,
                                                               int nparents, int shift, unsigned mask, int nb, const unsigned* __restrict__ toffs,
                                                               unsigned long long* __restrict__ out_keys, unsigned* __restrict__ out_rows,
                                                               unsigned* __restrict__ out_bucket) {
  __shared__ unsigned s_cnt[kMaxNb2], s_start[kMaxNb2], s_goff[kMaxNb2], s_wsum[kThreads / 64];
  __shared__ unsigned s_a[kThreads], s_b[kThreads];
  __shared__ unsigned long long s_stage[kMsTile];
  __shared__ uint16_t s_bin[kMsTile];
  __shared__ int s_pick;
  __shared__ unsigned s_carry;
  const TileRange r = ms_tile(pstart, nparents, n, s_a, s_b, s_wsum, &s_pick);
  if (r.parent < 0) return;
  const int t = threadIdx.x;
  for (int b = t; b < nb; b += kThreads) s_cnt[b] = 0;
  unsigned long long k[kMsRows];
  unsigned rw[kMsRows], bk[kMsRows], dg[kMsRows], rank[kMsRows];
  bool live[kMsRows];
#pragma unroll
  for (int u = 0; u < kMsRows; u++) {
    const int64_t i = r.lo + u * kThreads + t;
    live[u] = i < r.hi;
    k[u] = live[u] ? __builtin_nontemporal_load(&keys[i]) : 0ull;
    rw[u] = live[u] ? __builtin_nontemporal_load(&rows[i]) : 0u;
    bk[u] = live[u] ? __builtin_nontemporal_load(&bucket[i]) : 0u;
  }
  __syncthreads();
#pragma unroll
  for (int u = 0; u < kMsRows; u++) {
    dg[u] = (bk[u] >> shift) & mask;
    rank[u] = live[u] ? atomicAdd(&s_cnt[dg[u]], 1u) : 0u;
  }
  __syncthreads();
  digit_excl_scan(s_cnt, nb, s_a, s_b, s_wsum, &s_carry, [&](int d, unsigned st) {
    s_start[d] = st;
    s_goff[d] = toffs[r.id * nb + d] - st;
  });
  const int tile_n = (int)(r.hi - r.lo);
#pragma unroll
  for (int u = 0; u < kMsRows; u++)
    if (live[u]) { const unsigned q = s_start[dg[u]] + rank[u]; s_stage[q] = k[u]; s_bin[q] = (uint16_t)dg[u]; }
  __syncthreads();
  int64_t dst[kMsRows];
#pragma unroll
  for (int u = 0; u < kMsRows; u++) {
    const int q = u * kThreads + t;
    dst[u] = q < tile_n ? (int64_t)s_goff[s_bin[q]] + q : -1;
    if (dst[u] >= 0) out_keys[dst[u]] = s_stage[q];
  }
  __syncthreads();
  unsigned* s_stage32 = reinterpret_cast<unsigned*>(s_stage);
#pragma unroll
  for (int u = 0; u < kMsRows; u++)
    if (live[u]) { const unsigned q = s_start[dg[u]] + rank[u]; s_stage32[q] = rw[u]; if (WITH_BUCKET) s_stage32[kMsTile + q] = bk[u]; }
  __syncthreads();
#pragma unroll
  for (int u = 0; u < kMsRows; u++)
    if (dst[u] >= 0) {
      out_rows[dst[u]] = s_stage32[u * kThreads + t];
      if (WITH_BUCKET) out_bucket[dst[u]] = s_stage32[kMsTile + u * kThreads + t];
    }
}

struct KR {
  unsigned long long k;
  unsigned r;
  static __device__ __forceinline__ bool less(const KR& a, const KR& b) { return a.k < b.k || (a.k == b.k && a.r < b.r); }
  static __device__ __forceinline__ KR xchg(const KR& a, int j, int lane) {
    KR o;
    o.k = ((unsigned long long)ms_xor_lane((unsigned)(a.k >> 32), j, lane) << 32) | ms_xor_lane((unsigned)a.k, j, lane);
    o.r = ms_xor_lane(a.r, j, lane);
    return o;
  }
};
__device__ __forceinline__ bool kr_less(const KR& a, const KR& b) { return KR::less(a, b); }
struct C64 {
  unsigned long long c;
  static __device__ __forceinline__ bool less(const C64& a, const C64& b) { return a.c < b.c; }
  static __device__ __forceinline__ C64 xchg(const C64& a, int j, int lane) {
    C64 o;
    o.c = ((unsigned long long)ms_xor_lane((unsigned)(a.c >> 32), j, lane) << 32) | ms_xor_lane((unsigned)a.c, j, lane);
    return o;
  }
};
constexpr int kMsRowBits = 27;
template <int SLOTS>
__device__ __forceinline__ void ms_sort_bucket(const unsigned long long* __restrict__ keys, const unsigned* rows, unsigned s, int m,
                                               int lane, unsigned* out_rows, unsigned long long* __restrict__ out64) {
  KR x[SLOTS];
#pragma unroll
  for (int sl = 0; sl < SLOTS; sl++) {
    const int i = sl * 64 + lane;
    x[sl].k = i < m ? keys[s + i] : ~0ull;
    x[sl].r = i < m ? rows[s + i] : ~0u;
  }
  auto emit = [&](int i, unsigned row) { if (i < m) { if (out64) out64[s + i] = row; else out_rows[s + i] = row; } };
  if (SLOTS <= 2) {
    const unsigned long long k0 = ((unsigned long long)__builtin_amdgcn_readfirstlane((unsigned)(x[0].k >> 32)) << 32) |
                                  __builtin_amdgcn_readfirstlane((unsigned)x[0].k);
    bool fits1 = true, fits2 = true;
#pragma unroll
    for (int sl = 0; sl < SLOTS; sl++) {
      const bool in = sl * 64 + lane < m;
      fits1 = fits1 && (!in || x[sl].k - k0 + (1ull << 36) < (1ull << 37));
      fits2 = fits2 && (!in || x[sl].k - k0 + (1ull << 56) < (1ull << 57));
    }
    if (__all(fits1)) {
      C64 y[SLOTS];
#pragma unroll
      for (int sl = 0; sl < SLOTS; sl++)
        y[sl].c = sl * 64 + lane < m ? ((x[sl].k - k0 + (1ull << 36)) << kMsRowBits) | x[sl].r : ~0ull;
      ms_bitonic<C64, SLOTS>(y, lane);
#pragma unroll
      for (int sl = 0; sl < SLOTS; sl++) emit(sl * 64 + lane, (unsigned)y[sl].c & ((1u << kMsRowBits) - 1u));
      return;
    }
    if (__all(fits2)) {
      C64 y[SLOTS];
#pragma unroll
      for (int sl = 0; sl < SLOTS; sl++)
        y[sl].c = sl * 64 + lane < m ? ((x[sl].k - k0 + (1ull << 56)) << 7) | (unsigned)(sl * 64 + lane) : ~0ull;
      ms_bitonic<C64, SLOTS>(y, lane);
      bool tie = false;
#pragma unroll
      for (int sl = 0; sl < SLOTS; sl++) {
        unsigned long long nxt = __shfl_down(y[sl].c, 1, 64);
        if (sl + 1 < SLOTS) {
          const unsigned long long head = ((unsigned long long)__builtin_amdgcn_readfirstlane((unsigned)(y[sl + 1 < SLOTS ? sl + 1 : sl].c >> 32)) << 32) |
                                          __builtin_amdgcn_readfirstlane((unsigned)y[sl + 1 < SLOTS ? sl + 1 : sl].c);
          nxt = lane == 63 ? head : nxt;
        } else if (lane == 63) {
          nxt = ~0ull;
        }
        tie = tie || (sl * 64 + lane + 1 < m && (y[sl].c >> 7) == (nxt >> 7));
      }
      if (!__any(tie)) {
#pragma unroll
        for (int sl = 0; sl < SLOTS; sl++) {
          const unsigned at = (unsigned)y[sl].c & 127u;
          unsigned row = __shfl(x[0].r, (int)(at & 63u), 64);
          if (SLOTS > 1) { const unsigned row1 = __shfl(x[SLOTS > 1 ? 1 : 0].r, (int)(at & 63u), 64); row = (at >> 6) ? row1 : row; }
          emit(sl * 64 + lane, row);
        }
        return;
      }
    }
  }
  ms_bitonic<KR, SLOTS>(x, lane);
#pragma unroll
  for (int sl = 0; sl < SLOTS; sl++) emit(sl * 64 + lane, x[sl].r);
}

__global__ __launch_bounds__(256) void ms_local_kernel(const unsigned long long* __restrict__ keys, const unsigned* rows,
                                                        const unsigned* __restrict__ bstart, int64_t nbuckets, unsigned* out_rows,
                                                        unsigned long long* __restrict__ out64, unsigned* __restrict__ oversize,
                                                        unsigned* __restrict__ big_list) {
  const int lane = threadIdx.x & 63;
  const int64_t b = (int64_t)blockIdx.x * 4 + (threadIdx.x >> 6);
  if (b >= nbuckets) return;
  const unsigned s = bstart[b], e = bstart[b + 1];
  const int m = (int)(e - s);
  if (m <= 0) return;
  if (m > kLocalMax) {
    if (lane == 0) {
      if (m > kBigMax) atomicMax(&oversize[0], (unsigned)m);
      else { const unsigned at = atomicAdd(&oversize[1], 1u); if (at < (unsigned)kBigList) big_list[at] = (unsigned)b; }
    }
    return;
  }
  if (m == 1) { if (lane == 0) { if (out64) out64[s] = rows[s]; else out_rows[s] = rows[s]; } return; }
  if (m <= 64) ms_sort_bucket<1>(keys, rows, s, m, lane, out_rows, out64);
  else if (m <= 128) ms_sort_bucket<2>(keys, rows, s, m, lane, out_rows, out64);
  else if (m <= 256) ms_sort_bucket<4>(keys, rows, s, m, lane, out_rows, out64);
  else ms_sort_bucket<8>(keys, rows, s, m, lane, out_rows, out64);
}

__global__ __launch_bounds__(kThreads) void ms_big_kernel(const unsigned long long* __restrict__ keys, const unsigned* rows,
                                                           const unsigned* __restrict__ bstart, const unsigned* __restrict__ oversize,
                                                           const unsigned* __restrict__ big_list, unsigned* out_rows,
                                                           unsigned long long* __restrict__ out64) {
  __shared__ unsigned long long s_k[kBigMax];
  __shared__ unsigned s_r[kBigMax];
  if (blockIdx.x >= oversize[1] || blockIdx.x >= (unsigned)kBigList) return;
  const unsigned b = big_list[blockIdx.x], s = bstart[b];
  const int m = (int)(bstart[b + 1] - s);
  int p2 = 1024;
  while (p2 < m) p2 <<= 1;
  for (int i = threadIdx.x; i < p2; i += kThreads) { s_k[i] = i < m ? keys[s + i] : ~0ull; s_r[i] = i < m ? rows[s + i] : ~0u; }
  __syncthreads();
  for (int k = 2; k <= p2; k <<= 1) {
    for (int j = k >> 1; j > 0; j >>= 1) {
      for (int i = threadIdx.x; i < p2; i += kThreads) {
        const int q = i ^ j;
        if (q > i) {
          const KR x{s_k[i], s_r[i]}, y{s_k[q], s_r[q]};
          const bool asc = (i & k) == 0;
          if (kr_less(y, x) == asc) { s_k[i] = y.k; s_r[i] = y.r; s_k[q] = x.k; s_r[q] = x.r; }
        }
      }
      __syncthreads();
    }
  }
  for (int i = threadIdx.x; i < m; i += kThreads) { if (out64) out64[s + i] = s_r[i]; else out_rows[s + i] = s_r[i]; }
}

}

static void ms_plan(int64_t n, int* lb_out, int* lb2_out) {
  int lb = 0;
  while (((int64_t)64 << lb) < n) lb++;
  if (lb > 21) lb = 21;
  *lb_out = lb;
  *lb2_out = lb >= 20 ? lb - 10 : lb - lb / 2;
}

size_t ah_sort_msd_temp_bytes(int64_t n) {
  if (n < ((int64_t)1 << 22) || n > ((int64_t)1 << 27)) return 0;
  int lb, lb2;
  ms_plan(n, &lb, &lb2);
  const int nb2 = 1 << lb2, nb1 = 1 << (lb - lb2);
  const int64_t ntiles = ah_ceil_div(n, kMsTile), ngrp = ah_ceil_div(ntiles, kGroupTiles), nvt = ((ntiles + nb1 + 7) / 8) * 8;
  return ah_pad((size_t)n * 4) * 2 + ah_pad((size_t)kSample * 8) * 2 + ah_pad((size_t)kSample * 4) * 2 + ah_pad((size_t)(kSplit + 1) * 8) + ah_pad(kFlagWords * 4) + ah_pad(4097 * 2) +
         ah_pad((size_t)ntiles * nb1 * 4) * 2 + ah_pad((size_t)ngrp * nb1 * 4) + ah_pad((size_t)(nb1 + 1) * 4) + ah_pad((size_t)nvt * nb2 * 4) * 2 +
         ah_pad(((size_t)1 << lb) * 4 + 4) + ah_pad((size_t)kBigList * 4) + 256;
}

int ah_sort_rest_msd(ah_ctx* c, unsigned long long* keys, unsigned* rows, unsigned long long* alt_keys, unsigned* alt_rows, int64_t n,
                     unsigned long long varying, unsigned long long kmin, unsigned long long kmax, int float_bytes, int descending, void* tmp,
                     unsigned long long* out64, int* used) {
  *used = -1;
  if (!tmp || varying == 0 || ah_sort_msd_temp_bytes(n) == 0) return AH_OK;
  unsigned* out_rows = rows;
  int lb, lb2;
  ms_plan(n, &lb, &lb2);
  const int nb2 = 1 << lb2, nb1 = 1 << (lb - lb2);
  const unsigned nbuckets = 1u << lb;
  const int hb = 63 - __builtin_clzll(varying);
  MsMap map{hb == 63 ? ~0ull : ((1ull << (hb + 1)) - 1), 63 - hb, float_bytes, descending};
  const int64_t ntiles = ah_ceil_div(n, kMsTile), ngrp = ah_ceil_div(ntiles, kGroupTiles), nvt = ((ntiles + nb1 + 7) / 8) * 8;
  const unsigned grid1 = (unsigned)(((ntiles + 7) / 8) * 8);
  const int64_t sample_n = n < kSample ? n : kSample;
  TempCarver tc;
  tc.base = (uint8_t*)tmp;
  int rc;
  unsigned* bucket = (unsigned*)tc.take((size_t)n * 4);
  unsigned* bucket2 = (unsigned*)tc.take((size_t)n * 4);
  unsigned long long* sample = (unsigned long long*)tc.take((size_t)kSample * 8);
  unsigned long long* sample_alt = (unsigned long long*)tc.take((size_t)kSample * 8);
  unsigned* sample_rows = (unsigned*)tc.take((size_t)kSample * 4);
  unsigned* sample_rows_alt = (unsigned*)tc.take((size_t)kSample * 4);
  unsigned long long* split = (unsigned long long*)tc.take((size_t)(kSplit + 1) * 8);
  unsigned* flags = (unsigned*)tc.take(kFlagWords * 4);
  unsigned short* guide = (unsigned short*)tc.take(4097 * 2);
  unsigned* cnt1 = (unsigned*)tc.take((size_t)ntiles * nb1 * 4);
  unsigned* toffs1 = (unsigned*)tc.take((size_t)ntiles * nb1 * 4);
  unsigned* gsum = (unsigned*)tc.take((size_t)ngrp * nb1 * 4);
  unsigned* pstart = (unsigned*)tc.take((size_t)(nb1 + 1) * 4);
  unsigned* cnt2 = (unsigned*)tc.take((size_t)nvt * nb2 * 4);
  unsigned* toffs2 = (unsigned*)tc.take((size_t)nvt * nb2 * 4);
  unsigned* bstart = (unsigned*)tc.take(((size_t)nbuckets + 1) * 4);
  unsigned* big_list = (unsigned*)tc.take((size_t)kBigList * 4);
  unsigned* oversize = (unsigned*)&c->dscalars[26];
  AH_HIP(c, hipMemsetAsync(oversize, 0, 8, c->stream));
  ms_sample_kernel<<<(unsigned)ah_ceil_div(sample_n, 256), 256, 0, c->stream>>>(keys, n, n / sample_n, sample_n, map, sample, sample_rows);
  AH_LAUNCH_CHECK(c);
  unsigned long long* sorted = nullptr;
  if ((rc = ah_sort_pairs_lsd(c, sample, sample_rows, sample_alt, sample_rows_alt, sample_n, (unsigned*)cnt2, (unsigned*)toffs2, &sorted)) != AH_OK) return rc;
  {
    const int64_t run = (int64_t)(kBigMax / 2) * sample_n / n;
    ms_dupes_kernel<<<(unsigned)ah_ceil_div(sample_n, 256), 256, 0, c->stream>>>(sorted, sample_n, run < 1 ? 1 : run, oversize);
    AH_LAUNCH_CHECK(c);
    AH_HIP(c, hipMemcpyAsync(&c->pinned[12], oversize, 8, hipMemcpyDeviceToHost, c->stream));
    AH_HIP(c, hipStreamSynchronize(c->stream));
    if (((volatile unsigned*)&c->pinned[12])[0] != 0) {
      if (getenv("ARROWHIP_DEBUG_MSD")) fprintf(stderr, "msd: n=%lld: the sample shows a key with more than %d rows, not attempted\n", (long long)n, kBigMax / 2);
      *used = -1;
      return AH_OK;
    }
  }
  *used = 0;
  MsPoints pts{sorted, sample_n, (kmin & map.mask) << map.lshift, (kmax & map.mask) << map.lshift};
  AH_HIP(c, hipMemsetAsync(flags, 0, kFlagWords * 4, c->stream));
  ms_split_kernel<<<(kSplit + 256) / 256, 256, 0, c->stream>>>(pts, split, flags);
  AH_LAUNCH_CHECK(c);
  ms_guide_kernel<<<17, 256, 0, c->stream>>>(split, guide);
  AH_LAUNCH_CHECK(c);
  ms_bucket_kernel<<<ah_stream_grid(c, ah_ceil_div(n, kThreads * 4), 2), kThreads, 0, c->stream>>>(keys, n, map, pts, split, flags, guide, nbuckets / kSplit, bucket);
  AH_LAUNCH_CHECK(c);
  tile_hist_kernel<MsDigit><<<grid1, kThreads, 0, c->stream>>>(MsDigit{bucket, lb2, (unsigned)(nb1 - 1)}, n, nullptr, 1, nb1, cnt1);
  AH_LAUNCH_CHECK(c);
  if ((rc = launch_tile_offsets(c, cnt1, nb1, ntiles, n, gsum, toffs1, pstart)) != AH_OK) return rc;
  ms_scatter_kernel<true><<<grid1, kThreads, 0, c->stream>>>(keys, rows, bucket, n, nullptr, 1, lb2, (unsigned)(nb1 - 1), nb1, toffs1, alt_keys,
                                                                        alt_rows, bucket2);
  AH_LAUNCH_CHECK(c);
  tile_hist_kernel<MsDigit><<<(unsigned)nvt, kThreads, 0, c->stream>>>(MsDigit{bucket2, 0, (unsigned)(nb2 - 1)}, n, pstart, nb1, nb2, cnt2);
  AH_LAUNCH_CHECK(c);
  ms_offs2_kernel<<<(unsigned)nb1, kThreads, 0, c->stream>>>(cnt2, pstart, nb1, nb2, toffs2, bstart, n);
  AH_LAUNCH_CHECK(c);
  ms_scatter_kernel<false><<<(unsigned)nvt, kThreads, 0, c->stream>>>(alt_keys, alt_rows, bucket2, n, pstart, nb1, 0, (unsigned)(nb2 - 1), nb2, toffs2, keys,
                                                                      rows, nullptr);
  AH_LAUNCH_CHECK(c);
  ms_local_kernel<<<(unsigned)ah_ceil_div((int64_t)nbuckets, 4), 256, 0, c->stream>>>(keys, rows, bstart, (int64_t)nbuckets, out_rows, out64, oversize, big_list);
  AH_LAUNCH_CHECK(c);
  ms_big_kernel<<<kBigList, kThreads, 0, c->stream>>>(keys, rows, bstart, oversize, big_list, out_rows, out64);
  AH_LAUNCH_CHECK(c);
  AH_HIP(c, hipMemcpyAsync(&c->pinned[12], oversize, 8, hipMemcpyDeviceToHost, c->stream));
  AH_HIP(c, hipStreamSynchronize(c->stream));
  const unsigned too_big = ((volatile unsigned*)&c->pinned[12])[0], listed = ((volatile unsigned*)&c->pinned[12])[1];
  if (getenv("ARROWHIP_DEBUG_MSD")) fprintf(stderr, "msd: n=%lld lb=%d nb1=%d nb2=%d largest unsortable bucket=%u, buckets sorted by a workgroup=%u\n", (long long)n, lb, nb1, nb2, too_big, listed);
  if (too_big != 0 || listed > (unsigned)kBigList) return AH_OK;
  *used = 1;
  return AH_OK;
}
```

arrow_go_amd/csrc/ah_sort_radix.h:

```cpp
#pragma once
#include <algorithm>
#include <vector>
#include "ah_common.h"
#include "ah_reduce.h"

namespace {

constexpr int kBlock = 256;
constexpr int kWaves = kBlock / 64;
constexpr int kItems = 8;
constexpr int kTile = kBlock * kItems;
constexpr int kRadix = 256;
constexpr int kAndOrGrid = 4096;
constexpr int kMaxTilesPerBlock = 8;

static inline int tiles_per_block(int64_t n) { return n >= ((int64_t)1 << 24) ? kMaxTilesPerBlock : 1; }

struct Pairs {
  const unsigned long long* keys;
  const unsigned* rows;
  int shift;
  __device__ __forceinline__ void load(int64_t i, unsigned long long* key, unsigned* row, unsigned* digit) const {
    *key = keys[i];
    *row = rows[i];
    *digit = (unsigned)(*key >> shift) & 255u;
  }
};

template <typename SRC>
__global__ __launch_bounds__(kBlock) void hist_kernel(SRC src, int64_t n, unsigned* __restrict__ hist, int64_t nblocks, int tpb) {
  __shared__ unsigned s_h[kWaves][kRadix];
  for (int i = threadIdx.x; i < kWaves * kRadix; i += kBlock) (&s_h[0][0])[i] = 0;
  __syncthreads();
  const int lane = threadIdx.x & 63, wave = threadIdx.x >> 6;
  const int64_t block = blockIdx.x;
  for (int t = 0; t < tpb; t++) {
    const int64_t wbase = (block * tpb + t) * kTile + (int64_t)wave * (kItems * 64);
    if (wbase >= n) break;
#pragma unroll
    for (int r = 0; r < kItems; r++) {
      const int64_t i = wbase + r * 64 + lane;
      if (i < n) {
        unsigned long long key; unsigned row, digit;
        src.load(i, &key, &row, &digit);
        atomicAdd(&s_h[wave][digit], 1u);
      }
    }
  }
  __syncthreads();
  for (int d = threadIdx.x; d < kRadix; d += kBlock) {
    unsigned t = 0;
#pragma unroll
    for (int w = 0; w < kWaves; w++) t += s_h[w][d];
    hist[(int64_t)d * nblocks + block] = t;
  }
}

template <typename SRC>
__global__ __launch_bounds__(kBlock) void scatter_kernel(SRC src, int64_t n, const unsigned* __restrict__ hist, const unsigned* __restrict__ offs,
                                                          int64_t nblocks, int tpb, unsigned long long* __restrict__ out_keys,
                                                          unsigned* __restrict__ out_rows) {
  __shared__ unsigned s_cnt[kWaves][kRadix];
  __shared__ unsigned s_start[kRadix], s_goff[kRadix], s_wsum[kWaves];
  __shared__ unsigned long long s_keys[kTile];
  __shared__ unsigned s_rows[kTile];
  __shared__ uint8_t s_dig[kTile];
  static_assert(kBlock == kRadix, "one thread per digit in the prefix step");
  const int lane = threadIdx.x & 63, wave = threadIdx.x >> 6;
  unsigned run_d = offs[(int64_t)threadIdx.x * nblocks + blockIdx.x] - hist[(int64_t)threadIdx.x * nblocks + blockIdx.x];
  for (int tb = 0; tb < tpb; tb++) {
  const int64_t tile = (int64_t)blockIdx.x * tpb + tb;
  if (tile * kTile >= n) break;
  for (int i = threadIdx.x; i < kWaves * kRadix; i += kBlock) (&s_cnt[0][0])[i] = 0;
  __syncthreads();
  const int64_t wbase = tile * kTile + (int64_t)wave * (kItems * 64);
  unsigned long long key[kItems];
  unsigned row[kItems], digit[kItems], rank[kItems];
  bool live[kItems];
#pragma unroll
  for (int r = 0; r < kItems; r++) {
    const int64_t i = wbase + r * 64 + lane;
    live[r] = i < n;
    key[r] = 0; row[r] = 0; digit[r] = 0;
    if (live[r]) src.load(i, &key[r], &row[r], &digit[r]);
  }
  const unsigned long long below = lane == 0 ? 0ull : (~0ull >> (64 - lane));
#pragma unroll
  for (int r = 0; r < kItems; r++) {
    unsigned long long peers = __ballot(live[r]);
#pragma unroll
    for (int b = 0; b < 8; b++) {
      const unsigned long long bal = __ballot((digit[r] >> b) & 1u);
      peers &= ((digit[r] >> b) & 1u) ? bal : ~bal;
    }
    if (live[r]) {
      unsigned* cnt = &s_cnt[wave][digit[r]];
      const unsigned before = __hip_atomic_load(cnt, __ATOMIC_RELAXED, __HIP_MEMORY_SCOPE_WAVEFRONT);
      rank[r] = before + (unsigned)__popcll(peers & below);
      if ((peers & below) == 0)
        __hip_atomic_store(cnt, before + (unsigned)__popcll(peers), __ATOMIC_RELAXED, __HIP_MEMORY_SCOPE_WAVEFRONT);
    }
    __builtin_amdgcn_fence(__ATOMIC_SEQ_CST, "wavefront");
    __builtin_amdgcn_wave_barrier();
  }
  __syncthreads();
  unsigned tot = 0;
  {
    const int d = threadIdx.x;
#pragma unroll
    for (int w = 0; w < kWaves; w++) {
      const unsigned t = s_cnt[w][d];
      s_cnt[w][d] = tot;
      tot += t;
    }
    unsigned inc = tot;
#pragma unroll
    for (int o = 1; o < 64; o <<= 1) {
      const unsigned t = __shfl_up(inc, o, 64);
      if (lane >= o) inc += t;
    }
    if (lane == 63) s_wsum[wave] = inc;
    __syncthreads();
    unsigned wbase = 0;
#pragma unroll
    for (int w = 0; w < kWaves; w++) if (w < wave) wbase += s_wsum[w];
    const unsigned start = wbase + inc - tot;
    s_start[d] = start;
    s_goff[d] = run_d - start;
    run_d += tot;
  }
  __syncthreads();
#pragma unroll
  for (int r = 0; r < kItems; r++) {
    if (live[r]) {
      const unsigned lp = s_start[digit[r]] + s_cnt[wave][digit[r]] + rank[r];
      s_keys[lp] = key[r];
      s_rows[lp] = row[r];
      s_dig[lp] = (uint8_t)digit[r];
    }
  }
  __syncthreads();
  const int64_t tile_n = n - tile * kTile >= kTile ? kTile : n - tile * kTile;
  for (int lp = threadIdx.x; lp < tile_n; lp += kBlock) {
    const unsigned pos = s_goff[s_dig[lp]] + (unsigned)lp;
    out_keys[pos] = s_keys[lp];
    out_rows[pos] = s_rows[lp];
  }
  }
}

struct KeyStats {
  unsigned long long a, o, mn, mx, nans;
  __device__ __forceinline__ void init() { a = ~0ull; o = 0ull; mn = ~0ull; mx = 0ull; nans = 0; }
  __device__ __forceinline__ void add(unsigned long long k) { a &= k; o |= k; mn = k < mn ? k : mn; mx = k > mx ? k : mx; }
  __device__ __forceinline__ void merge(const KeyStats& p) {
    a &= p.a; o |= p.o;
    mn = p.mn < mn ? p.mn : mn;
    mx = p.mx > mx ? p.mx : mx;
    nans += p.nans;
  }
  template <int NWORDS>
  __device__ __forceinline__ void store(unsigned long long* res) const {
    res[0] = a; res[1] = o; res[2] = mn; res[3] = mx;
    if (NWORDS == 5) res[4] = nans;
  }
};

__global__ __launch_bounds__(kBlock) void and_or_kernel(const unsigned long long* __restrict__ keys, int64_t n, unsigned long long* __restrict__ res) {
  KeyStats st;
  st.init();
  const int64_t stride = (int64_t)gridDim.x * kBlock;
  for (int64_t i = (int64_t)blockIdx.x * kBlock + threadIdx.x; i < n; i += stride) st.add(keys[i]);
  st = ah_block_reduce<kBlock>(st);
  if (threadIdx.x == 0) st.store<4>(res + (size_t)blockIdx.x * 4);
}

struct Carver {
  uint8_t* base;
  size_t used = 0;
  static size_t pad(size_t b) { return (b + 255) & ~(size_t)255; }
  template <typename P>
  void take(size_t bytes, P** out) { *out = (P*)(base + used); used += pad(bytes); }
};

template <typename SRC>
int radix_pass(ah_ctx* c, SRC src, int64_t n, unsigned* hist, unsigned* offs, unsigned long long* out_keys, unsigned* out_rows) {
  const int tpb = tiles_per_block(n);
  const int64_t nblocks = ah_ceil_div(n, (int64_t)kTile * tpb);
  hist_kernel<SRC><<<(unsigned)nblocks, kBlock, 0, c->stream>>>(src, n, hist, nblocks, tpb);
  AH_LAUNCH_CHECK(c);
  int rc = ah_cumulative_sum(c, AH_UINT32, hist, nullptr, 0, (int64_t)kRadix * nblocks, nullptr, 0, 0, offs, nullptr, nullptr);
  if (rc != AH_OK) return rc;
  scatter_kernel<SRC><<<(unsigned)nblocks, kBlock, 0, c->stream>>>(src, n, hist, offs, nblocks, tpb, out_keys, out_rows);
  AH_LAUNCH_CHECK(c);
  return AH_OK;
}

}

struct SortCol {
  int type;
  const void* values;
  const void* offsets;
  const uint8_t* data;
  int width;
  const uint8_t* valid;
  int64_t off;
  int descending, nulls_at_start;
};

constexpr int kBinArrays = 8;

struct SortBuffers {
  void* msd_tmp = nullptr;
  uint64_t* final_out = nullptr;
  bool emitted = false;
  unsigned long long *ka, *kb, *andor;
  unsigned *ra, *rb, *rc;
  unsigned *hist, *offs;
  unsigned* bin[kBinArrays] = {};
};

bool ah_sort_is_binary(int type);
int ah_sort_by_binary(ah_ctx* c, SortBuffers& b, const SortCol& col, int64_t n, const unsigned* rows_in);
```

Baseline: 6529.

## Process multiple tiles per workgroup in MSD sort and store second digit as uint16

The MSD radix sort passes now let each workgroup handle a slice of several tiles, looping with a prefetch of the next tile's digits. This shrinks the per-tile count and offset tables. The first scatter writes a compact 16-bit second-level digit array instead of a full 32-bit bucket copy, which cuts the bytes the second pass reads. A precomputed tile table replaces the per-block parent search in the second histogram. This only affects sort, not the measured Sum/Add/Filter/Take kernels, and with default slice settings the gain depends on ms_slice_tiles.

```diff
diff --git a/arrow_go_amd/csrc/ah_common.h b/arrow_go_amd/csrc/ah_common.h
--- a/arrow_go_amd/csrc/ah_common.h
+++ b/arrow_go_amd/csrc/ah_common.h
@@ -56,6 +56,7 @@
   int opt_hash_direct;
   int opt_hash_sum_partition;
   int opt_sort_msd;
+  int opt_sort_slice_tiles;
   int opt_scan_segment_log2;
   void* expr_cache;
   int capturing;
@@ -149,8 +150,8 @@
                           unsigned long long* out_vals, unsigned* out_ids);
 int ah_sort_rest_msd(ah_ctx* ctx, unsigned long long* keys, unsigned* rows, unsigned long long* alt_keys, unsigned* alt_rows, int64_t n,
                      unsigned long long varying, unsigned long long kmin, unsigned long long kmax, int float_bytes, int descending, void* tmp,
-                     unsigned long long* out64, int* used);
-size_t ah_sort_msd_temp_bytes(int64_t n);
+                     size_t tmp_bytes, unsigned long long* out64, int* used);
+size_t ah_sort_msd_temp_bytes(const ah_ctx* ctx, int64_t n, int slice_tiles = 0);
 int ah_sort_pairs_lsd(ah_ctx* ctx, unsigned long long* keys, unsigned* rows, unsigned long long* alt_keys, unsigned* alt_rows, int64_t n,
                       unsigned* hist, unsigned* offs, unsigned long long** sorted_keys);
 int ah_take_binned_try(ah_ctx* ctx, int byte_width, const void* values, const uint8_t* vvalid, int64_t voff, int64_t nvalues, int iw,
diff --git a/arrow_go_amd/csrc/ah_ctx.hip b/arrow_go_amd/csrc/ah_ctx.hip
--- a/arrow_go_amd/csrc/ah_ctx.hip
+++ b/arrow_go_amd/csrc/ah_ctx.hip
@@ -44,6 +44,7 @@
   c->opt_encode_byte_map = env_int("ARROWHIP_ENCODE_BYTE_MAP", 1);
   c->opt_encode_part_slots = env_int("ARROWHIP_ENCODE_PART_SLOTS", 8192);
   c->opt_sort_msd = env_int("ARROWHIP_SORT_MSD", 1);
+  c->opt_sort_slice_tiles = env_int("ARROWHIP_SORT_SLICE_TILES", 0);
   c->opt_scan_segment_log2 = env_int("ARROWHIP_SCAN_SEGMENT_LOG2", 0);
   c->opt_take_gather_lds = env_int("ARROWHIP_TAKE_GATHER_LDS", 1);
   c->opt_take_vec_nt = env_int("ARROWHIP_TAKE_VEC_NT", 7);
@@ -147,6 +148,7 @@
   else if (!strcmp(name, "encode_byte_map")) c->opt_encode_byte_map = (int)value;
   else if (!strcmp(name, "encode_part_slots")) c->opt_encode_part_slots = (int)value;
   else if (!strcmp(name, "sort_msd")) c->opt_sort_msd = (int)value;
+  else if (!strcmp(name, "sort_slice_tiles")) c->opt_sort_slice_tiles = value < 0 ? 0 : (int)value;
   else if (!strcmp(name, "scan_onepass")) c->opt_scan_onepass = (int)value;
   else if (!strcmp(name, "groupby_lean")) c->opt_groupby_lean = (int)value;
   else if (!strcmp(name, "groupby_seed")) c->opt_groupby_seed = (int)value;
diff --git a/arrow_go_amd/csrc/ah_msd.h b/arrow_go_amd/csrc/ah_msd.h
--- a/arrow_go_amd/csrc/ah_msd.h
+++ b/arrow_go_amd/csrc/ah_msd.h
@@ -9,15 +9,19 @@
 constexpr int kMaxNb2 = 2048;
 
 struct TileRange { int64_t lo, hi, id; int parent; };
+__device__ __forceinline__ int64_t ms_uniform(int64_t v) {
+  return (int64_t)(((unsigned long long)(unsigned)__builtin_amdgcn_readfirstlane((int)((unsigned long long)v >> 32)) << 32) |
+                   (unsigned)__builtin_amdgcn_readfirstlane((int)(unsigned)v));
+}
 __device__ __forceinline__ int ms_parent_of(int j, int nparents) { const int per = nparents >> 3; return ((j % per) << 3) | (j / per); }
-__device__ __forceinline__ unsigned ms_tiles_of(const unsigned* __restrict__ pstart, const unsigned* __restrict__ pend, int j, int nparents) {
+__device__ __forceinline__ unsigned ms_tiles_of(const unsigned* __restrict__ pstart, const unsigned* __restrict__ pend, int j, int nparents, int unit = kMsTile) {
   const int p = ms_parent_of(j, nparents);
-  return ((pend ? pend[p] : pstart[p + 1]) - pstart[p] + kMsTile - 1) / kMsTile;
+  return ((pend ? pend[p] : pstart[p + 1]) - pstart[p] + (unsigned)unit - 1) / (unsigned)unit;
 }
 __device__ __forceinline__ void ms_parent_tiles(const unsigned* __restrict__ pstart, const unsigned* __restrict__ pend, int nparents, unsigned* s_cnt,
-                                                unsigned* s_start, unsigned* s_wsum) {
+                                                unsigned* s_start, unsigned* s_wsum, int unit = kMsTile) {
   const int t = threadIdx.x;
-  s_cnt[t] = t < nparents ? ms_tiles_of(pstart, pend, t, nparents) : 0u;
+  s_cnt[t] = t < nparents ? ms_tiles_of(pstart, pend, t, nparents, unit) : 0u;
   __syncthreads();
   block_excl_scan(s_cnt, s_start, s_wsum, nparents);
 }
@@ -40,38 +44,38 @@
   return g;
 }
 __device__ __forceinline__ TileRange ms_tile_of_parent(const unsigned* __restrict__ pstart, const unsigned* __restrict__ pend, int nparents, int j, long long g,
-                                                       const unsigned* s_start) {
+                                                       const unsigned* s_start, int unit = kMsTile) {
   TileRange r;
   const int p = ms_parent_of(j, nparents);
   const int64_t b0 = pstart[p], b1 = pend ? pend[p] : pstart[p + 1];
-  r.lo = b0 + (int64_t)(g - s_start[j]) * kMsTile;
-  r.hi = r.lo + kMsTile < b1 ? r.lo + kMsTile : b1;
+  r.lo = b0 + (int64_t)(g - s_start[j]) * unit;
+  r.hi = r.lo + unit < b1 ? r.lo + unit : b1;
   r.id = g;
   r.parent = p;
   return r;
 }
 __device__ __forceinline__ TileRange ms_tile(const unsigned* __restrict__ pstart, int nparents, int64_t n, unsigned* s_cnt, unsigned* s_start,
-                                             unsigned* s_wsum, int* s_pick, const unsigned* __restrict__ pend = nullptr) {
+                                             unsigned* s_wsum, int* s_pick, const unsigned* __restrict__ pend = nullptr, int unit = kMsTile) {
   TileRange r{0, 0, 0, -1};
   if (!pstart) {
-    const int64_t tile = xcd_contiguous_tile((n + kMsTile - 1) / kMsTile);
-    if (tile >= 0) { r.lo = tile * kMsTile; r.hi = r.lo + kMsTile < n ? r.lo + kMsTile : n; r.id = tile; r.parent = 0; }
+    const int64_t tile = xcd_contiguous_tile((n + unit - 1) / unit);
+    if (tile >= 0) { r.lo = tile * unit; r.hi = r.lo + unit < n ? r.lo + unit : n; r.id = tile; r.parent = 0; }
     return r;
   }
   const int t = threadIdx.x;
   if (t == 0) *s_pick = -1;
-  ms_parent_tiles(pstart, pend, nparents, s_cnt, s_start, s_wsum);
+  ms_parent_tiles(pstart, pend, nparents, s_cnt, s_start, s_wsum, unit);
   const long long g = ms_block_tile(blockIdx.x, gridDim.x, nparents, s_cnt, s_start);
   if (g >= 0 && t < nparents && s_cnt[t] && s_start[t] <= g && g < s_start[t] + s_cnt[t]) *s_pick = t;
   __syncthreads();
   const int j = *s_pick;
-  return j < 0 ? r : ms_tile_of_parent(pstart, pend, nparents, j, g, s_start);
+  return j < 0 ? r : ms_tile_of_parent(pstart, pend, nparents, j, g, s_start, unit);
 }
 
 __global__ __launch_bounds__(kThreads) void ms_tile_table_kernel(const unsigned* __restrict__ pstart, const unsigned* __restrict__ pend, int nparents,
-                                                                  unsigned nblocks, TileRange* __restrict__ table) {
+                                                                  unsigned nblocks, TileRange* __restrict__ table, int unit = kMsTile) {
   __shared__ unsigned s_cnt[kThreads], s_start[kThreads], s_wsum[kThreads / 64];
-  ms_parent_tiles(pstart, pend, nparents, s_cnt, s_start, s_wsum);
+  ms_parent_tiles(pstart, pend, nparents, s_cnt, s_start, s_wsum, unit);
   const unsigned b = blockIdx.x * (unsigned)kThreads + threadIdx.x;
   if (b >= nblocks) return;
   const long long g = ms_block_tile(b, nblocks, nparents, s_cnt, s_start);
@@ -81,26 +85,49 @@
     while (lo < hi) { const int mid = (lo + hi + 1) >> 1; if ((long long)s_start[mid] <= g) lo = mid; else hi = mid - 1; }
     int j = lo;
     while (j > 0 && !s_cnt[j]) j--;
-    if (s_cnt[j] && (long long)s_start[j] <= g && g < (long long)s_start[j] + s_cnt[j]) r = ms_tile_of_parent(pstart, pend, nparents, j, g, s_start);
+    if (s_cnt[j] && (long long)s_start[j] <= g && g < (long long)s_start[j] + s_cnt[j]) r = ms_tile_of_parent(pstart, pend, nparents, j, g, s_start, unit);
   }
   table[b] = r;
 }
 
-template <typename DIGIT>
+template <typename DIGIT, bool SLICES = false>
 __global__ __launch_bounds__(kThreads) void tile_hist_kernel(DIGIT dg, int64_t n, const unsigned* __restrict__ pstart, int nparents, int nb,
-                                                              unsigned* __restrict__ cnt, const TileRange* __restrict__ tile_table = nullptr) {
+                                                              unsigned* __restrict__ cnt, const TileRange* __restrict__ tile_table = nullptr,
+                                                              int unit = kMsTile) {
   __shared__ unsigned s_h[DIGIT::kMaxDigits];
   __shared__ unsigned s_cnt[kThreads], s_start[kThreads], s_wsum[kThreads / 64];
   __shared__ int s_pick;
-  const TileRange r = tile_table ? tile_table[blockIdx.x] : ms_tile(pstart, nparents, n, s_cnt, s_start, s_wsum, &s_pick);
+  const TileRange r = tile_table ? tile_table[blockIdx.x] : ms_tile(pstart, nparents, n, s_cnt, s_start, s_wsum, &s_pick, nullptr, SLICES ? unit : kMsTile);
   if (r.parent < 0) return;
   for (int b = threadIdx.x; b < nb; b += kThreads) s_h[b] = 0;
   __syncthreads();
   unsigned d[kMsRows];
-#pragma unroll
-  for (int u = 0; u < kMsRows; u++) { const int64_t i = r.lo + u * kThreads + threadIdx.x; d[u] = i < r.hi ? dg.digit(i, r.parent) : 0u; }
-#pragma unroll
-  for (int u = 0; u < kMsRows; u++) { const int64_t i = r.lo + u * kThreads + threadIdx.x; if (i < r.hi) atomicAdd(&s_h[d[u]], 1u); }
+  if constexpr (SLICES) {
+    const int64_t hi = ms_uniform(r.hi);
+    const int parent = __builtin_amdgcn_readfirstlane(r.parent);
+    int64_t lo = ms_uniform(r.lo);
+#pragma unroll
+    for (int u = 0; u < kMsRows; u++) { const int64_t i = lo + u * kThreads + threadIdx.x; d[u] = i < hi ? dg.digit(i, parent) : 0u; }
+    for (;;) {
+      const int64_t next = lo + kMsTile;
+      unsigned e[kMsRows];
+      if (next < hi) {
+#pragma unroll
+        for (int u = 0; u < kMsRows; u++) { const int64_t i = next + u * kThreads + threadIdx.x; e[u] = i < hi ? dg.digit(i, parent) : 0u; }
+      }
+#pragma unroll
+      for (int u = 0; u < kMsRows; u++) { const int64_t i = lo + u * kThreads + threadIdx.x; if (i < hi) atomicAdd(&s_h[d[u]], 1u); }
+      if (next >= hi) break;
+#pragma unroll
+      for (int u = 0; u < kMsRows; u++) d[u] = e[u];
+      lo = next;
+    }
+  } else {
+#pragma unroll
+    for (int u = 0; u < kMsRows; u++) { const int64_t i = r.lo + u * kThreads + threadIdx.x; d[u] = i < r.hi ? dg.digit(i, r.parent) : 0u; }
+#pragma unroll
+    for (int u = 0; u < kMsRows; u++) { const int64_t i = r.lo + u * kThreads + threadIdx.x; if (i < r.hi) atomicAdd(&s_h[d[u]], 1u); }
+  }
   __syncthreads();
   for (int b = threadIdx.x; b < nb; b += kThreads) cnt[r.id * nb + b] = s_h[b];
 }
@@ -108,11 +135,11 @@
 __global__ __launch_bounds__(kThreads) void ms_offs2_kernel(const unsigned* __restrict__ cnt, const unsigned* __restrict__ pstart, int nparents, int nb,
                                                              unsigned* __restrict__ toffs, unsigned* __restrict__ bstart, int64_t n,
                                                              unsigned* __restrict__ largest = nullptr, unsigned* __restrict__ done = nullptr,
-                                                             unsigned long long* mb = nullptr, unsigned long long seq = 0) {
+                                                             unsigned long long* mb = nullptr, unsigned long long seq = 0, int unit = kMsTile) {
   __shared__ unsigned s_cnt[kThreads], s_start[kThreads], s_wsum[kThreads / 64];
   __shared__ unsigned s_carry;
   const int t = threadIdx.x, p = blockIdx.x;
-  ms_parent_tiles(pstart, nullptr, nparents, s_cnt, s_start, s_wsum);
+  ms_parent_tiles(pstart, nullptr, nparents, s_cnt, s_start, s_wsum, unit);
   const int j = (p & 7) * (nparents >> 3) + (p >> 3);
   const int64_t vt0 = s_start[j], vt1 = vt0 + s_cnt[j];
   __syncthreads();
diff --git a/arrow_go_amd/csrc/ah_sort.hip b/arrow_go_amd/csrc/ah_sort.hip
--- a/arrow_go_amd/csrc/ah_sort.hip
+++ b/arrow_go_amd/csrc/ah_sort.hip
@@ -160,11 +160,11 @@
     if (rows_in == nullptr && nvar >= 4 && c->opt_sort_msd) {
       int used = -1;
       if ((rc = ah_sort_rest_msd(c, kcur, rcur, kalt, ralt, rest_n, varying, kmin, kmax, std::is_floating_point<T>::value ? (int)sizeof(T) : 0, descending, b.msd_tmp,
-                                 (unsigned long long*)(rest_n == n ? b.final_out : nullptr), &used)) != AH_OK) return rc;
+                                 b.msd_tmp_bytes, (unsigned long long*)(rest_n == n ? b.final_out : nullptr), &used)) != AH_OK) return rc;
       if (used > 0) {
         done = true;
         b.emitted = rest_n == n && b.final_out != nullptr;
-      } else if (used == 0 && b.msd_tmp && ah_sort_msd_temp_bytes(rest_n) != 0) {
+      } else if (used == 0 && b.msd_tmp && ah_sort_msd_temp_bytes(c, rest_n) != 0) {
         if ((rc = radix_pass(c, col, n, b.hist, b.offs, b.ka, b.ra)) != AH_OK) return rc;
       }
     }
@@ -199,7 +199,7 @@
   bool any_binary = false;
   for (int k = 0; k < nkeys; k++) any_binary |= ah_sort_is_binary(keys[k].type);
   const size_t hist_bytes = (size_t)kRadix * ntiles * 4;
-  const size_t msd_bytes = c->opt_sort_msd ? ah_sort_msd_temp_bytes(n) : 0;
+  const size_t msd_bytes = c->opt_sort_msd ? ah_sort_msd_temp_bytes(c, n) : 0;
   const size_t bin_bytes = any_binary ? kBinArrays * Carver::pad((size_t)n * 4) : 0;
   const size_t total = 2 * Carver::pad((size_t)n * 8) + (nkeys > 1 ? 3 : 2) * Carver::pad((size_t)n * 4) + 2 * Carver::pad(hist_bytes) + Carver::pad(4096 * 8 * 8) + Carver::pad(msd_bytes) + bin_bytes;
   void* arena;
@@ -214,7 +214,7 @@
   tmp.take(hist_bytes, &b.hist);
   tmp.take(hist_bytes, &b.offs);
   tmp.take((size_t)kAndOrGrid * 8 * 8, &b.andor);
-  if (msd_bytes) { uint8_t* m; tmp.take(msd_bytes, &m); b.msd_tmp = m; }
+  if (msd_bytes) { uint8_t* m; tmp.take(msd_bytes, &m); b.msd_tmp = m; b.msd_tmp_bytes = msd_bytes; }
   if (any_binary)
     for (int i = 0; i < kBinArrays; i++) tmp.take((size_t)n * 4, &b.bin[i]);
   const unsigned* rows_in = nullptr;
diff --git a/arrow_go_amd/csrc/ah_sort_msd.hip b/arrow_go_amd/csrc/ah_sort_msd.hip
--- a/arrow_go_amd/csrc/ah_sort_msd.hip
+++ b/arrow_go_amd/csrc/ah_sort_msd.hip
@@ -151,69 +151,102 @@
   const unsigned* bucket; int shift; unsigned mask;
   __device__ __forceinline__ unsigned digit(int64_t i, int) const { return (__builtin_nontemporal_load(&bucket[i]) >> shift) & mask; }
 };
+struct MsDigit16 {
+  static constexpr int kMaxDigits = kMaxNb2;
+  const uint16_t* digit2;
+  __device__ __forceinline__ unsigned digit(int64_t i, int) const { return __builtin_nontemporal_load(&digit2[i]); }
+};
 
 template <bool WITH_BUCKET>
 __global__ __launch_bounds__(kThreads) void ms_scatter_kernel(const unsigned long long* __restrict__ keys, const unsigned* __restrict__ rows,
-                                                               const unsigned* __restrict__ bucket, int64_t n, const unsigned* __restrict__ pstart,
-                                                               int nparents, int shift, unsigned mask, int nb, const unsigned* __restrict__ toffs,
-                                                               unsigned long long* __restrict__ out_keys, unsigned* __restrict__ out_rows,
-                                                               unsigned* __restrict__ out_bucket) {
+                                                               const std::conditional_t<WITH_BUCKET, unsigned, uint16_t>* __restrict__ bucket, int64_t n,
+                                                               const unsigned* __restrict__ pstart, int nparents, int shift, unsigned mask, int nb,
+                                                               const unsigned* __restrict__ toffs, unsigned long long* __restrict__ out_keys,
+                                                               unsigned* __restrict__ out_rows, uint16_t* __restrict__ out_bucket, unsigned keep, int unit) {
   __shared__ unsigned s_cnt[kMaxNb2], s_start[kMaxNb2], s_goff[kMaxNb2], s_wsum[kThreads / 64];
   __shared__ unsigned s_a[kThreads], s_b[kThreads];
   __shared__ unsigned long long s_stage[kMsTile];
   __shared__ uint16_t s_bin[kMsTile];
   __shared__ int s_pick;
-  __shared__ unsigned s_carry;
-  const TileRange r = ms_tile(pstart, nparents, n, s_a, s_b, s_wsum, &s_pick);
+  const TileRange r = ms_tile(pstart, nparents, n, s_a, s_b, s_wsum, &s_pick, nullptr, unit);
   if (r.parent < 0) return;
-  const int t = threadIdx.x;
-  for (int b = t; b < nb; b += kThreads) s_cnt[b] = 0;
-  unsigned long long k[kMsRows];
-  unsigned rw[kMsRows], bk[kMsRows], dg[kMsRows], rank[kMsRows];
-  bool live[kMsRows];
-#pragma unroll
-  for (int u = 0; u < kMsRows; u++) {
-    const int64_t i = r.lo + u * kThreads + t;
-    live[u] = i < r.hi;
-    k[u] = live[u] ? __builtin_nontemporal_load(&keys[i]) : 0ull;
-    rw[u] = live[u] ? __builtin_nontemporal_load(&rows[i]) : 0u;
-    bk[u] = live[u] ? __builtin_nontemporal_load(&bucket[i]) : 0u;
-  }
-  __syncthreads();
-#pragma unroll
-  for (int u = 0; u < kMsRows; u++) {
-    dg[u] = (bk[u] >> shift) & mask;
-    rank[u] = live[u] ? atomicAdd(&s_cnt[dg[u]], 1u) : 0u;
-  }
-  __syncthreads();
-  digit_excl_scan(s_cnt, nb, s_a, s_b, s_wsum, &s_carry, [&](int d, unsigned st) {
-    s_start[d] = st;
-    s_goff[d] = toffs[r.id * nb + d] - st;
-  });
-  const int tile_n = (int)(r.hi - r.lo);
-#pragma unroll
-  for (int u = 0; u < kMsRows; u++)
-    if (live[u]) { const unsigned q = s_start[dg[u]] + rank[u]; s_stage[q] = k[u]; s_bin[q] = (uint16_t)dg[u]; }
-  __syncthreads();
-  int64_t dst[kMsRows];
-#pragma unroll
-  for (int u = 0; u < kMsRows; u++) {
-    const int q = u * kThreads + t;
-    dst[u] = q < tile_n ? (int64_t)s_goff[s_bin[q]] + q : -1;
-    if (dst[u] >= 0) out_keys[dst[u]] = s_stage[q];
-  }
-  __syncthreads();
+  int t = threadIdx.x;
+  const unsigned slice_lo = (unsigned)__builtin_amdgcn_readfirstlane((int)r.lo), slice_hi = (unsigned)__builtin_amdgcn_readfirstlane((int)r.hi);
+  const unsigned* __restrict__ toffs_row = toffs + (int64_t)__builtin_amdgcn_readfirstlane((int)r.id) * nb;
   unsigned* s_stage32 = reinterpret_cast<unsigned*>(s_stage);
-#pragma unroll
-  for (int u = 0; u < kMsRows; u++)
-    if (live[u]) { const unsigned q = s_start[dg[u]] + rank[u]; s_stage32[q] = rw[u]; if (WITH_BUCKET) s_stage32[kMsTile + q] = bk[u]; }
-  __syncthreads();
-#pragma unroll
-  for (int u = 0; u < kMsRows; u++)
-    if (dst[u] >= 0) {
-      out_rows[dst[u]] = s_stage32[u * kThreads + t];
-      if (WITH_BUCKET) out_bucket[dst[u]] = s_stage32[kMsTile + u * kThreads + t];
-    }
+  static_assert(kMaxNb2 == 2 * kThreads, "a thread owns digits 2t and 2t + 1");
+  for (unsigned lo = slice_lo; lo < slice_hi; lo += kMsTile) {
+    asm volatile("" : "+v"(t));
+    const int lane = t & 63, wave = t >> 6;
+    const int tile_n = (int)(slice_hi - lo < (unsigned)kMsTile ? slice_hi - lo : (unsigned)kMsTile);
+    const bool own = 2 * t < nb;
+    if (own) { s_cnt[2 * t] = 0; s_cnt[2 * t + 1] = 0; }
+    unsigned long long k[kMsRows];
+    unsigned rw[kMsRows], bk[kMsRows], rank[kMsRows];
+#pragma unroll
+    for (int u = 0; u < kMsRows; u++) {
+      const int q = u * kThreads + t < tile_n ? u * kThreads + t : tile_n - 1;
+      k[u] = __builtin_nontemporal_load(&keys[lo + q]);
+      rw[u] = __builtin_nontemporal_load(&rows[lo + q]);
+      bk[u] = __builtin_nontemporal_load(&bucket[lo + q]);
+    }
+    if (lo == slice_lo && own) { s_goff[2 * t] = toffs_row[2 * t]; s_goff[2 * t + 1] = toffs_row[2 * t + 1]; }
+    __syncthreads();
+    auto digit = [&](int u) { return WITH_BUCKET ? (bk[u] >> shift) & mask : bk[u]; };
+#pragma unroll
+    for (int u = 0; u < kMsRows; u++) rank[u] = u * kThreads + t < tile_n ? atomicAdd(&s_cnt[digit(u)], 1u) : 0u;
+    __syncthreads();
+    {
+      const unsigned c0 = own ? s_cnt[2 * t] : 0u, c1 = own ? s_cnt[2 * t + 1] : 0u;
+      unsigned inc = c0 + c1;
+#pragma unroll
+      for (int o = 1; o < 64; o <<= 1) {
+        const unsigned v = (unsigned)__builtin_amdgcn_ds_bpermute(((lane - o) & 63) << 2, (int)inc);
+        if (lane >= o) inc += v;
+      }
+      if (lane == 63) s_wsum[wave] = inc;
+      __syncthreads();
+      unsigned base = (lane & 15) < wave ? s_wsum[lane & 15] : 0u;
+#pragma unroll
+      for (int j = 1; j < 16; j <<= 1) base += ms_xor_lane(base, j, lane);
+      const unsigned st0 = base + inc - (c0 + c1), st1 = st0 + c0;
+      if (own) {
+        s_start[2 * t] = st0; s_start[2 * t + 1] = st1;
+        s_goff[2 * t] -= st0; s_goff[2 * t + 1] -= st1;
+      }
+      __syncthreads();
+    }
+#pragma unroll
+    for (int u = 0; u < kMsRows; u++)
+      if (u * kThreads + t < tile_n) { const unsigned q = s_start[digit(u)] + rank[u]; s_stage[q] = k[u]; s_bin[q] = (uint16_t)digit(u); }
+    __syncthreads();
+    unsigned dst[kMsRows];
+#pragma unroll
+    for (int u = 0; u < kMsRows; u++) {
+      const int q = u * kThreads + t;
+      dst[u] = q < tile_n ? s_goff[s_bin[q]] + (unsigned)q : 0u;
+      if (q < tile_n) out_keys[dst[u]] = s_stage[q];
+    }
+    __syncthreads();
+    if (lo + kMsTile < slice_hi && own) {
+      s_goff[2 * t] += s_start[2 * t] + s_cnt[2 * t];
+      s_goff[2 * t + 1] += s_start[2 * t + 1] + s_cnt[2 * t + 1];
+    }
+#pragma unroll
+    for (int u = 0; u < kMsRows; u++)
+      if (u * kThreads + t < tile_n) {
+        const unsigned q = s_start[digit(u)] + rank[u];
+        s_stage32[q] = rw[u];
+        if (WITH_BUCKET) s_stage32[kMsTile + q] = bk[u] & keep;
+      }
+    __syncthreads();
+#pragma unroll
+    for (int u = 0; u < kMsRows; u++)
+      if (u * kThreads + t < tile_n) {
+        out_rows[dst[u]] = s_stage32[u * kThreads + t];
+        if (WITH_BUCKET) out_bucket[dst[u]] = (uint16_t)s_stage32[kMsTile + u * kThreads + t];
+      }
+  }
 }
 
 struct KR {
@@ -368,22 +401,40 @@
   *lb2_out = lb >= 20 ? lb - 10 : lb - lb / 2;
 }
 
-size_t ah_sort_msd_temp_bytes(int64_t n) {
+static int ms_slice_tiles(const ah_ctx* c) { return c->opt_sort_slice_tiles >= 1 ? c->opt_sort_slice_tiles : 1; }
+static size_t ms_table2_bytes(int64_t nvt, int nb2) {
+  const size_t table = (size_t)nvt * nb2 * 4, lsd = (size_t)256 * (size_t)ah_ceil_div(kSample, 2048) * 4;
+  return table > lsd ? table : lsd;
+}
+struct MsSlices { int unit; int64_t n1, ngrp, nvt; };
+static MsSlices ms_slices(int64_t n, int nb1, int slice_tiles) {
+  MsSlices s;
+  const int64_t ntiles = ah_ceil_div(n, kMsTile);
+  s.unit = (int)(slice_tiles < ntiles ? slice_tiles : ntiles) * kMsTile;
+  s.n1 = ah_ceil_div(n, s.unit);
+  s.ngrp = ah_ceil_div(s.n1, kGroupTiles);
+  s.nvt = ((s.n1 + nb1 + 7) / 8) * 8;
+  return s;
+}
+
+size_t ah_sort_msd_temp_bytes(const ah_ctx* c, int64_t n, int slice_tiles) {
   if (n < ((int64_t)1 << 22) || n > ((int64_t)1 << 27)) return 0;
   int lb, lb2;
   ms_plan(n, &lb, &lb2);
   const int nb2 = 1 << lb2, nb1 = 1 << (lb - lb2);
-  const int64_t ntiles = ah_ceil_div(n, kMsTile), ngrp = ah_ceil_div(ntiles, kGroupTiles), nvt = ((ntiles + nb1 + 7) / 8) * 8;
-  return ah_pad((size_t)n * 4) * 2 + ah_pad((size_t)kSample * 8) * 2 + ah_pad((size_t)kSample * 4) * 2 + ah_pad((size_t)(kSplit + 1) * 8) + ah_pad(kFlagWords * 4) + ah_pad(4097 * 2) +
-         ah_pad((size_t)ntiles * nb1 * 4) * 2 + ah_pad((size_t)ngrp * nb1 * 4) + ah_pad((size_t)(nb1 + 1) * 4) + ah_pad((size_t)nvt * nb2 * 4) * 2 +
-         ah_pad(((size_t)1 << lb) * 4 + 4) + ah_pad((size_t)kBigList * 4) + 256;
+  const MsSlices sl = ms_slices(n, nb1, slice_tiles >= 1 ? slice_tiles : ms_slice_tiles(c));
+  return ah_pad((size_t)n * 4) + ah_pad((size_t)n * 2) + ah_pad((size_t)kSample * 8) * 2 + ah_pad((size_t)kSample * 4) * 2 + ah_pad((size_t)(kSplit + 1) * 8) + ah_pad(kFlagWords * 4) + ah_pad(4097 * 2) +
+         ah_pad((size_t)sl.n1 * nb1 * 4) * 2 + ah_pad((size_t)sl.ngrp * nb1 * 4) + ah_pad((size_t)(nb1 + 1) * 4) + ah_pad(ms_table2_bytes(sl.nvt, nb2)) * 2 +
+         ah_pad((size_t)sl.nvt * sizeof(TileRange)) + ah_pad(((size_t)1 << lb) * 4 + 4) + ah_pad((size_t)kBigList * 4) + 256;
 }
 
 int ah_sort_rest_msd(ah_ctx* c, unsigned long long* keys, unsigned* rows, unsigned long long* alt_keys, unsigned* alt_rows, int64_t n,
                      unsigned long long varying, unsigned long long kmin, unsigned long long kmax, int float_bytes, int descending, void* tmp,
-                     unsigned long long* out64, int* used) {
+                     size_t tmp_bytes, unsigned long long* out64, int* used) {
   *used = -1;
-  if (!tmp || varying == 0 || ah_sort_msd_temp_bytes(n) == 0) return AH_OK;
+  if (!tmp || varying == 0 || ah_sort_msd_temp_bytes(c, n) == 0) return AH_OK;
+  const int slice_tiles = ms_slice_tiles(c);
+  if (ah_sort_msd_temp_bytes(c, n, slice_tiles) > tmp_bytes) return AH_OK;
   unsigned* out_rows = rows;
   int lb, lb2;
   ms_plan(n, &lb, &lb2);
@@ -391,14 +442,15 @@
   const unsigned nbuckets = 1u << lb;
   const int hb = 63 - __builtin_clzll(varying);
   MsMap map{hb == 63 ? ~0ull : ((1ull << (hb + 1)) - 1), 63 - hb, float_bytes, descending};
-  const int64_t ntiles = ah_ceil_div(n, kMsTile), ngrp = ah_ceil_div(ntiles, kGroupTiles), nvt = ((ntiles + nb1 + 7) / 8) * 8;
-  const unsigned grid1 = (unsigned)(((ntiles + 7) / 8) * 8);
+  const MsSlices sl = ms_slices(n, nb1, slice_tiles);
+  const int64_t nvt = sl.nvt;
+  const unsigned grid1 = (unsigned)(((sl.n1 + 7) / 8) * 8);
   const int64_t sample_n = n < kSample ? n : kSample;
   TempCarver tc;
   tc.base = (uint8_t*)tmp;
   int rc;
   unsigned* bucket = (unsigned*)tc.take((size_t)n * 4);
-  unsigned* bucket2 = (unsigned*)tc.take((size_t)n * 4);
+  uint16_t* digit2 = (uint16_t*)tc.take((size_t)n * 2);
   unsigned long long* sample = (unsigned long long*)tc.take((size_t)kSample * 8);
   unsigned long long* sample_alt = (unsigned long long*)tc.take((size_t)kSample * 8);
   unsigned* sample_rows = (unsigned*)tc.take((size_t)kSample * 4);
@@ -406,12 +458,13 @@
   unsigned long long* split = (unsigned long long*)tc.take((size_t)(kSplit + 1) * 8);
   unsigned* flags = (unsigned*)tc.take(kFlagWords * 4);
   unsigned short* guide = (unsigned short*)tc.take(4097 * 2);
-  unsigned* cnt1 = (unsigned*)tc.take((size_t)ntiles * nb1 * 4);
-  unsigned* toffs1 = (unsigned*)tc.take((size_t)ntiles * nb1 * 4);
-  unsigned* gsum = (unsigned*)tc.take((size_t)ngrp * nb1 * 4);
+  unsigned* cnt1 = (unsigned*)tc.take((size_t)sl.n1 * nb1 * 4);
+  unsigned* toffs1 = (unsigned*)tc.take((size_t)sl.n1 * nb1 * 4);
+  unsigned* gsum = (unsigned*)tc.take((size_t)sl.ngrp * nb1 * 4);
   unsigned* pstart = (unsigned*)tc.take((size_t)(nb1 + 1) * 4);
-  unsigned* cnt2 = (unsigned*)tc.take((size_t)nvt * nb2 * 4);
-  unsigned* toffs2 = (unsigned*)tc.take((size_t)nvt * nb2 * 4);
+  unsigned* cnt2 = (unsigned*)tc.take(ms_table2_bytes(nvt, nb2));
+  unsigned* toffs2 = (unsigned*)tc.take(ms_table2_bytes(nvt, nb2));
+  TileRange* tiles2 = (TileRange*)tc.take((size_t)nvt * sizeof(TileRange));
   unsigned* bstart = (unsigned*)tc.take(((size_t)nbuckets + 1) * 4);
   unsigned* big_list = (unsigned*)tc.take((size_t)kBigList * 4);
   unsigned* oversize = (unsigned*)&c->dscalars[26];
@@ -441,18 +494,20 @@
   AH_LAUNCH_CHECK(c);
   ms_bucket_kernel<<<ah_stream_grid(c, ah_ceil_div(n, kThreads * 4), 2), kThreads, 0, c->stream>>>(keys, n, map, pts, split, flags, guide, nbuckets / kSplit, bucket);
   AH_LAUNCH_CHECK(c);
-  tile_hist_kernel<MsDigit><<<grid1, kThreads, 0, c->stream>>>(MsDigit{bucket, lb2, (unsigned)(nb1 - 1)}, n, nullptr, 1, nb1, cnt1);
-  AH_LAUNCH_CHECK(c);
-  if ((rc = launch_tile_offsets(c, cnt1, nb1, ntiles, n, gsum, toffs1, pstart)) != AH_OK) return rc;
+  tile_hist_kernel<MsDigit, true><<<grid1, kThreads, 0, c->stream>>>(MsDigit{bucket, lb2, (unsigned)(nb1 - 1)}, n, nullptr, 1, nb1, cnt1, nullptr, sl.unit);
+  AH_LAUNCH_CHECK(c);
+  if ((rc = launch_tile_offsets(c, cnt1, nb1, sl.n1, n, gsum, toffs1, pstart)) != AH_OK) return rc;
   ms_scatter_kernel<true><<<grid1, kThreads, 0, c->stream>>>(keys, rows, bucket, n, nullptr, 1, lb2, (unsigned)(nb1 - 1), nb1, toffs1, alt_keys,
-                                                                        alt_rows, bucket2);
-  AH_LAUNCH_CHECK(c);
-  tile_hist_kernel<MsDigit><<<(unsigned)nvt, kThreads, 0, c->stream>>>(MsDigit{bucket2, 0, (unsigned)(nb2 - 1)}, n, pstart, nb1, nb2, cnt2);
-  AH_LAUNCH_CHECK(c);
-  ms_offs2_kernel<<<(unsigned)nb1, kThreads, 0, c->stream>>>(cnt2, pstart, nb1, nb2, toffs2, bstart, n);
-  AH_LAUNCH_CHECK(c);
-  ms_scatter_kernel<false><<<(unsigned)nvt, kThreads, 0, c->stream>>>(alt_keys, alt_rows, bucket2, n, pstart, nb1, 0, (unsigned)(nb2 - 1), nb2, toffs2, keys,
-                                                                      rows, nullptr);
+                                                                        alt_rows, digit2, (unsigned)(nb2 - 1), sl.unit);
+  AH_LAUNCH_CHECK(c);
+  ms_tile_table_kernel<<<(unsigned)ah_ceil_div(nvt, kThreads), kThreads, 0, c->stream>>>(pstart, nullptr, nb1, (unsigned)nvt, tiles2, sl.unit);
+  AH_LAUNCH_CHECK(c);
+  tile_hist_kernel<MsDigit16, true><<<(unsigned)nvt, kThreads, 0, c->stream>>>(MsDigit16{digit2}, n, pstart, nb1, nb2, cnt2, tiles2, sl.unit);
+  AH_LAUNCH_CHECK(c);
+  ms_offs2_kernel<<<(unsigned)nb1, kThreads, 0, c->stream>>>(cnt2, pstart, nb1, nb2, toffs2, bstart, n, nullptr, nullptr, nullptr, 0, sl.unit);
+  AH_LAUNCH_CHECK(c);
+  ms_scatter_kernel<false><<<(unsigned)nvt, kThreads, 0, c->stream>>>(alt_keys, alt_rows, digit2, n, pstart, nb1, 0, (unsigned)(nb2 - 1), nb2, toffs2, keys,
+                                                                      rows, nullptr, 0u, sl.unit);
   AH_LAUNCH_CHECK(c);
   ms_local_kernel<<<(unsigned)ah_ceil_div((int64_t)nbuckets, 4), 256, 0, c->stream>>>(keys, rows, bstart, (int64_t)nbuckets, out_rows, out64, oversize, big_list);
   AH_LAUNCH_CHECK(c);
@@ -461,7 +516,7 @@
   AH_HIP(c, hipMemcpyAsync(&c->pinned[12], oversize, 8, hipMemcpyDeviceToHost, c->stream));
   AH_HIP(c, hipStreamSynchronize(c->stream));
   const unsigned too_big = ((volatile unsigned*)&c->pinned[12])[0], listed = ((volatile unsigned*)&c->pinned[12])[1];
-  if (getenv("ARROWHIP_DEBUG_MSD")) fprintf(stderr, "msd: n=%lld lb=%d nb1=%d nb2=%d largest unsortable bucket=%u, buckets sorted by a workgroup=%u\n", (long long)n, lb, nb1, nb2, too_big, listed);
+  if (getenv("ARROWHIP_DEBUG_MSD")) fprintf(stderr, "msd: n=%lld lb=%d nb1=%d nb2=%d tiles per slice=%d largest unsortable bucket=%u, buckets sorted by a workgroup=%u\n", (long long)n, lb, nb1, nb2, sl.unit / kMsTile, too_big, listed);
   if (too_big != 0 || listed > (unsigned)kBigList) return AH_OK;
   *used = 1;
   return AH_OK;
diff --git a/arrow_go_amd/csrc/ah_sort_radix.h b/arrow_go_amd/csrc/ah_sort_radix.h
--- a/arrow_go_amd/csrc/ah_sort_radix.h
+++ b/arrow_go_amd/csrc/ah_sort_radix.h
@@ -213,6 +213,7 @@
 
 struct SortBuffers {
   void* msd_tmp = nullptr;
+  size_t msd_tmp_bytes = 0;
   uint64_t* final_out = nullptr;
   bool emitted = false;
   unsigned long long *ka, *kb, *andor;
```

Result: slower. 6305 (-3.4%).
